# homenc/HElib

Hardware: AMD Instinct MI355X
Metric: ctxt_x_ctxt_mults_per_sec_incl_relinearize (higher is better)
Workload: dtype u64; 1 GPU; BGV m=32768 p=65537 bits=950 (L=16x60b, K=6x56b, 6 small primes, D=3): Ctxt::multiplyBy on FRESH ciphertexts = multLowLvl (bringToSet x2 + tensorProduct) + reLinearize (dropSmallAndSpecialPrimes + key switch), benchmarks/bgv_basic.cpp:144-165; added noise MEASURED as in the reference (device canonical-embedding norms, read back lazily); the loop is driven by the C++17 host (libhelib_amd_host.so); ; batch_per_gpu=128, pairs_all_ranks=128

## Files before the change

helib_amd/csrc/bgv_slots.hip:

```cpp
#include <hip/hip_runtime.h>

#include <cstdarg>
#include <cstdio>
#include <cstring>
#include <mutex>
#include <vector>

#include "../../include/helib_amd.h"
#include "bgv_slots.h"
#include "ckks_bridge.h"
#include "hostmath.h"
#include "prof.h"

struct hx_bgv_slots {
  hx_ctx* ctx = nullptr;
  hx_ctx* side = nullptr;
  uint64_t m = 0, p = 0, rho = 0, k = 0;
  uint32_t N = 0;
  int device = 0;
  std::vector<uint64_t> gens, ords;
  uint32_t* d_row2slot = nullptr;
  uint32_t* d_slot2row = nullptr;
  void* buf[3] = {nullptr, nullptr, nullptr};
  size_t cap[3] = {0, 0, 0};
// ... 76 lines not shown
    if (!best)
      break;
    gens.push_back(best);
    ords.push_back(largest);
    conj_classes(cl, best, m);
  }
}

int ensure_buf(hx_bgv_slots* t, hipStream_t st, int slot, size_t bytes)
{
  if (t->cap[slot] >= bytes)
    return HX_OK;
  CK(hipStreamSynchronize(st));
  hipFree(t->buf[slot]);
  t->buf[slot] = nullptr;
  t->cap[slot] = 0;
  CK(hipMalloc(&t->buf[slot], bytes));
  t->cap[slot] = bytes;
  return HX_OK;
}

struct Enter {
  hxi::CtxView v{};
  std::unique_lock<std::recursive_mutex> lk;
  int open(const hx_bgv_slots* t, const char* what)
  {
    RC(hxi::ctx_enter(t->ctx, &v));
    lk = std::unique_lock<std::recursive_mutex>(*v.mu);
    if (v.capturing)
      return err(HX_ERR_INVALID, "%s waits for the device and cannot be captured in a graph", what);
    return hx_ctx_set_stream(t->side, (void*)v.stream);
  }
};
struct DrainOnExit {
  hipStream_t st;
  ~DrainOnExit() { (void)hipStreamSynchronize(st); }
};
struct Drop {
  hx_poly* t;
  ~Drop() { hx_poly_destroy(t); }
};

unsigned blocks_for(size_t items)
{
  const size_t b = (items + 255) / 256;
  return (unsigned)std::min<size_t>(std::max<size_t>(b, 1), hx::BGV_MAX_BLOCKS);
}
bool aligned16(const void* a) { return ((uintptr_t)a & 15) == 0; }

int side_poly(const hx_bgv_slots* t, int batch, hx_poly** out)
{
  const int zero = 0;
  return hx_poly_create_uninit(t->side, batch, &zero, 1, out);
}

int gather_out(hx_bgv_slots* t, hipStream_t st, hx_poly* sp, size_t words, int64_t* slots_out)
{
  RC(ensure_buf(t, st, 2, words * 8));
  HX_LAUNCH(hx::bgv_gather_kernel, dim3(blocks_for(words)), dim3(256), 0, st, hxi::poly_rows_read(sp), t->d_slot2row, t->N,
            words, (int64_t*)t->buf[2]);
  CK(hipGetLastError());
  CK(hipMemcpyAsync(slots_out, t->buf[2], words * 8, hipMemcpyDeviceToHost, st));
  CK(hipStreamSynchronize(st));
  return HX_OK;
}

int launch_redmul(const hx_bgv_slots* t, hipStream_t st, const int64_t* src, size_t words, uint64_t f, uint64_t* dst)
{
  const uint64_t p = t->p, mu = (uint64_t)(((hxh::u128)1 << 64) / p), fs = hxh::shoup(f, p);
  if (words % 2 == 0 && aligned16(src) && aligned16(dst))
    HX_LAUNCH(hx::bgv_redmul_kernel<2>, dim3(blocks_for(words / 2)), dim3(256), 0, st, src, words, p, mu, f, fs, dst);
  else
    HX_LAUNCH(hx::bgv_redmul_kernel<1>, dim3(blocks_for(words)), dim3(256), 0, st, src, words, p, mu, f, fs, dst);
  CK(hipGetLastError());
  return HX_OK;
}

}

extern "C" int hx_bgv_slots_destroy(hx_bgv_slots* t)
{
  if (!t)
    return HX_OK;
  (void)hipSetDevice(t->device);
  if (t->side)
    hx_ctx_destroy(t->side);
  hipFree(t->d_row2slot);
  hipFree(t->d_slot2row);
  for (void* b : t->buf)
    hipFree(b);
  delete t;
  return HX_OK;
}

extern "C" int hx_bgv_slots_create(hx_ctx* ctx, uint64_t p, hx_bgv_slots** out)
{
  if (!ctx || !out)
    return err(HX_ERR_INVALID, "null argument");
  *out = nullptr;
  hxi::CtxView v{};
  RC(hxi::ctx_enter(ctx, &v));
  std::unique_lock<std::recursive_mutex> lk(*v.mu);
  if (v.capturing)
    return err(HX_ERR_INVALID, "hx_bgv_slots_create while a graph is being captured");
  const uint64_t m = v.m;
  if (p < 2 || p >= (1ull << 60) || !hxh::is_prime(p))
    return err(HX_ERR_INVALID, "the plaintext modulus p = %llu is not a prime below 2^60", (unsigned long long)p);
  if (m % p == 0)
    return err(HX_ERR_INVALID, "p = %llu divides m = %llu", (unsigned long long)p, (unsigned long long)m);
  if (p % m != 1) {
    uint64_t d = 1;
    for (uint64_t x = p % m; x != 1; x = x * (p % m) % m)
      d++;
    return err(HX_ERR_UNSUPPORTED,
               "d = ord_m(p) = %llu for p = %llu, m = %llu: only d = 1 (p = 1 mod m, slots in Z_p) is built",
               (unsigned long long)d, (unsigned long long)p, (unsigned long long)m);
  }
  const bool pow2 = (m & (m - 1)) == 0;
  if (pow2 ? (m < 16 || m > (1u << 17)) : (m < 3))
    return err(HX_ERR_UNSUPPORTED, "BGV slots on the device need a power-of-two m in [16, 2^17] or another m >= 3 (m = %llu)",
               (unsigned long long)m);
  if (!pow2 && m % 2 == 0 && (p - 1) % (2 * m) != 0)
    return err(HX_ERR_UNSUPPORTED, "even m = %llu that is not a power of two needs 2m | p - 1 (p = %llu)",
               (unsigned long long)m, (unsigned long long)p);
  hx_bgv_slots* t = new hx_bgv_slots();
  struct Guard {
    hx_bgv_slots* t;
    ~Guard() { hx_bgv_slots_destroy(t); }
  } guard{t};
  t->ctx = ctx;
  t->m = m;
  t->p = p;
  t->N = v.phim;
  t->device = v.device;
  RC(hx_ctx_create(&t->side, v.device, m));
  RC(hx_ctx_set_stream(t->side, (void*)v.stream));
  int pidx = -1;
  uint64_t root = 0;
  RC(hx_ctx_add_prime(t->side, p, 0, &pidx));
  RC(hx_ctx_prime(t->side, pidx, nullptr, &root));
  const uint64_t zeta = pow2 ? root : hxh::mulmod(root, root, p);
  std::vector<uint32_t> zidx(m, hx::BGV_NO_SLOT);
  uint32_t n = 0;
  uint64_t pw = 1;
  for (uint64_t j = 0; j < m; j++, pw = hxh::mulmod(pw, zeta, p))
    if (hxh::gcd(j, m) == 1) {
      zidx[j] = n++;
      if (pw > t->rho) {
        t->rho = pw;
        t->k = j;
      }
    }
  if (n != t->N || hxh::powmod(zeta, m, p) != 1)
    return err(HX_ERR_DEVICE, "internal: the transform's root for p = %llu is not an m-th root of unity", (unsigned long long)p);
  find_generators(m, t->gens, t->ords);
  uint64_t nslots = 1;
  for (uint64_t o : t->ords)
    nslots *= o;
  if (nslots != t->N)
    return err(HX_ERR_DEVICE, "internal: the hypercube of Z_%llu^* has %llu points, not phi(m)", (unsigned long long)m,
               (unsigned long long)nslots);
  std::vector<uint32_t> slot2row(t->N), row2slot(t->N, hx::BGV_NO_SLOT);
  const size_t ng = t->gens.size();
  std::vector<uint64_t> e(ng, 0), part(ng + 1, 1);
  for (uint32_t i = 0; i < t->N; i++) {
    const uint64_t ti = part[ng];
    const uint64_t pos = hxh::mulmod(t->k, hxh::invmod(ti, m), m);
// ... 169 lines not shown
```

helib_amd/csrc/conv_kernels.hip:

```cpp
#include "dev_common.h"
#include "conv_dev.h"
#include "ntt_kernel_util.h"
#include "prof.h"

namespace hx {

__device__ __forceinline__ uint64_t uniform_u64(uint64_t v)
{
  const uint32_t lo = (uint32_t)__builtin_amdgcn_readfirstlane((int)(uint32_t)v);
  const uint32_t hi = (uint32_t)__builtin_amdgcn_readfirstlane((int)(uint32_t)(v >> 32));
  return ((uint64_t)hi << 32) | lo;
}
__device__ __forceinline__ TW uniform_tw(const TW& t)
{
  TW r;
  r.w = uniform_u64(t.w);
  r.wp = uniform_u64(t.wp);
  return r;
}

template <uint32_t SRC, uint32_t DST>
struct ConvIO {
  static constexpr int LOAD_BOUND = 1;
  static constexpr bool LAZY_STORE = true;
// ... 97 lines not shown
  using RN = RowNTT<LOGN, AR>;
  uint64_t v[32];
  uint32_t nl[32];
  const unsigned w = wave_index();
  RN::template fwd<0>(fresh_tid(w), v, nl, lds, io, twf, q);
  __syncthreads();
  RN::template fwd<1>(fresh_tid(w), v, nl, lds, io, twf, q);
  __syncthreads();
  RN::template fwd<2>(fresh_tid(w), v, nl, lds, io, twf, q);
  __syncthreads();
  RN::template fwd<3>(fresh_tid(w), v, nl, lds, io, twf, q);
  __syncthreads();
  RN::template fwd<4>(fresh_tid(w), v, nl, lds, io, twf, q);
  __syncthreads();
  RN::template fwd<5>(fresh_tid(w), v, nl, lds, io, twf, q);
  __syncthreads();
  RN::template fwd<6>(fresh_tid(w), v, nl, lds, io, twf, q);
  __syncthreads();
  RN::template fwd<7>(fresh_tid(w), v, nl, lds, io, twf, q);
  __syncthreads();
  RN::template inv<0>(fresh_tid(w), v, nl, lds, io, twi, q);
  __syncthreads();
  RN::template inv<1>(fresh_tid(w), v, nl, lds, io, twi, q);
  __syncthreads();
  RN::template inv<2>(fresh_tid(w), v, nl, lds, io, twi, q);
  __syncthreads();
  RN::template inv<3>(fresh_tid(w), v, nl, lds, io, twi, q);
  __syncthreads();
  RN::template inv<4>(fresh_tid(w), v, nl, lds, io, twi, q);
  __syncthreads();
  RN::template inv<5>(fresh_tid(w), v, nl, lds, io, twi, q);
  __syncthreads();
  RN::template inv<6>(fresh_tid(w), v, nl, lds, io, twi, q);
  __syncthreads();
  RN::template inv<7>(fresh_tid(w), v, nl, lds, io, twi, q);
}

template <int LOGN, uint32_t SRC, uint32_t DST>
__global__ void __launch_bounds__(Geo<LOGN>::T, HX_NTT_MINWAVES(LOGN))
ntt_conv_kernel(ConvRowArgs A, ConvRows R, const PrimeDev* __restrict__ cprimes, const TW* __restrict__ tw_arena)
{
  extern __shared__ __attribute__((aligned(16))) uint32_t lds[];
  const unsigned wid = xcd_remap(blockIdx.x, gridDim.x);
  const unsigned b = wid % A.batch, u = wid / A.batch, ri = u / A.split, g = u % A.split;
  const PrimeDev* pd = cprimes + uniform_u16(R.pd, u);
  const BluePrimeDev* P = R.bp[ri];
  constexpr unsigned Q = Geo<LOGN>::N;
  ConvIO<SRC, DST> io;
  const size_t seg = (size_t)ri * A.batch + b;
  const size_t polyseg = ((size_t)uniform_u16(R.row, ri) * A.batch + b) * A.phim;
  io.src = SRC == CONV_SRC_REV ? A.in + seg * A.in_stride : A.in + polyseg;
  io.dst = DST == CONV_DST_SUB ? A.out + ((size_t)u * A.batch + b) * Q : A.out + polyseg;
  io.aux = DST == CONV_DST_FINAL ? A.aux + seg * A.aux_stride : nullptr;
  io.hat = R.hat[ri] + (size_t)g * Q;
  io.P = P;
  io.S = &R.cp[ri]->S;
  io.zidx = A.zidx;
  io.g = g;
  io.split = A.split;
  io.Q = Q;
  io.phim = A.phim;
  io.m = A.m;
  io.d = A.d;
  io.base = A.base;
  io.alias = A.alias;
  io.r2 = pd->r2;
  const QC q = make_qc(pd->q, pd->mu64);
  const TW* twf = tw_arena + pd->tw_fwd_off;
  const TW* twi = tw_arena + pd->tw_inv_off;
#ifndef HX_NO_PROTH
  if (pd->proth) {
    conv_body<LOGN, ArProth>(lds, io, reinterpret_cast<const TWM*>(twf), reinterpret_cast<const TWM*>(twi), q);
    return;
  }
#endif
  conv_body<LOGN, ArShoup>(lds, io, twf, twi, q);
}

template <int LOGN, uint32_t SRC, uint32_t DST>
static hipError_t launch_conv(const ConvRowArgs& A, const ConvRows& R, int nunits, const PrimeDev* cprimes,
                              const TW* tw_arena, hipStream_t st)
{
  constexpr size_t lds_bytes = (size_t)Geo<LOGN>::LDS_WORDS * 4;
  bool attr_set = false;
  if (!attr_set) {
    hipError_t e = hxp::dyn_lds((const void*)ntt_conv_kernel<LOGN, SRC, DST>,
                                       hipFuncAttributeMaxDynamicSharedMemorySize, (int)lds_bytes);
    if (e != hipSuccess)
      return e;
    attr_set = true;
  }
  HX_LAUNCH((ntt_conv_kernel<LOGN, SRC, DST>), dim3((unsigned)nunits * A.batch), dim3(Geo<LOGN>::T), lds_bytes, st, A, R,
            cprimes, tw_arena);
  return hipGetLastError();
}
template <int LOGN>
static hipError_t launch_conv_n(const ConvRowArgs& A, const ConvRows& R, int nunits, const PrimeDev* cprimes,
                                const TW* tw_arena, hipStream_t st)
{
  if (A.src_mode == CONV_SRC_BLUE_PRE && A.dst_mode == CONV_DST_SUB)
    return launch_conv<LOGN, CONV_SRC_BLUE_PRE, CONV_DST_SUB>(A, R, nunits, cprimes, tw_arena, st);
  if (A.src_mode == CONV_SRC_SCATTER && A.dst_mode == CONV_DST_SUB)
    return launch_conv<LOGN, CONV_SRC_SCATTER, CONV_DST_SUB>(A, R, nunits, cprimes, tw_arena, st);
  if (A.src_mode == CONV_SRC_REV && A.dst_mode == CONV_DST_SUB)
    return launch_conv<LOGN, CONV_SRC_REV, CONV_DST_SUB>(A, R, nunits, cprimes, tw_arena, st);
  if (A.src_mode == CONV_SRC_REV && A.dst_mode == CONV_DST_FINAL)
    return launch_conv<LOGN, CONV_SRC_REV, CONV_DST_FINAL>(A, R, nunits, cprimes, tw_arena, st);
  return hipErrorInvalidValue;
}
hipError_t launch_conv_rows(int logn, const ConvRowArgs& A, const ConvRows& R, int nunits, const PrimeDev* cprimes,
                            const TW* tw_arena, hipStream_t st)
{
  switch (logn) {
    case 13: return launch_conv_n<13>(A, R, nunits, cprimes, tw_arena, st);
    case 14: return launch_conv_n<14>(A, R, nunits, cprimes, tw_arena, st);
    case 15: return launch_conv_n<15>(A, R, nunits, cprimes, tw_arena, st);
  }
  return hipErrorInvalidValue;
}

}
```

helib_amd/csrc/engine.hip:

```cpp
#include <hip/hip_runtime.h>

#include <cstdarg>
#include <cstdio>
#include <cstdlib>
#include <cstring>
#include <algorithm>
#include <chrono>
#include <map>
#include <mutex>
#include <string>
#include <unordered_set>
#include <vector>

#include "../../include/helib_amd.h"
#include "arena.h"
#include "prof.h"
#include "switches.h"
#include "dev_common.h"
#include "hostmath.h"
#include "bluestein.h"
#include "pfa_dev.h"
#include "rns_kernels.h"
#include "mfma_ext.h"
#include "rns_mfma_dev.h"
// ... 156 lines not shown
  uint64_t* scratch[11] = {nullptr, nullptr, nullptr, nullptr, nullptr, nullptr, nullptr, nullptr, nullptr, nullptr, nullptr};
  uint32_t* d_redo = nullptr;
  size_t redo_cap = 0;
  size_t scratch_words[11] = {0, 0, 0, 0, 0, 0, 0, 0, 0, 0, 0};
  uint64_t aux_q[3] = {0, 0, 0};
  int bk = 0, n1 = 0, n2 = 0, n3 = 0;
  uint32_t dq = 0, mpad = 0;
  PrimeDev* d_cprimes = nullptr;
  int ncprimes = 0, cprimes_cap = 0;
  std::vector<struct BluePrime*> blue;
  uint16_t* d_pfa_idx = nullptr;
  std::vector<ConvPlan> bigplan;
  std::vector<int64_t> psi_low, phi_coef;
  std::map<std::vector<uint64_t>, ExtPlan*> plans;
  hxa::SlabArena arena;
  std::unordered_set<struct hx_poly*> polys;
  int refs = 1;
  std::recursive_mutex mu;
  double* d_frac = nullptr;
  size_t frac_cap = 0, frac_pos = 0;
  bool want_frac = false;
  int xs_first = 0, xs_rows = 0;
  double xs_inv_qd = 0;
  bool want_fdelta = false;
  double2* d_wtab = nullptr;
  double2 *d_bn_v = nullptr, *d_bn_w = nullptr, *d_bn_chat = nullptr, *d_bn_Z = nullptr;
  size_t bn_rows_cap = 0;
  unsigned long long* d_norm2 = nullptr;
  size_t norm_cap = 0;
  double2* d_norm_park = nullptr;
  size_t norm_park_cap = 0;
  struct NormPending {
    hipEvent_t ev;
    unsigned long long* pinned;
    size_t cap;
    int rows;
    double* out;
    bool slab;
  };
  std::vector<void*> norm_slabs;
  bool defer_norms = false;
  std::vector<NormPending> norm_pending, norm_free;
  hipStream_t norm_stream = nullptr;
  hipEvent_t norm_in_ev = nullptr, norm_out_ev = nullptr;
  bool norm_reads_xs = false, norm_reads_frac = false;
  hipEvent_t timer[2] = {nullptr, nullptr};
  bool capturing = false;
  int graphs_alive = 0;
  hipStream_t own_stream = nullptr;
  std::vector<void*> graph_retired;
  void* ckks = nullptr;
  void (*ckks_free)(void*) = nullptr;
  void* linalg = nullptr;
  void (*linalg_free)(void*) = nullptr;
};

struct hx_poly {
  hx_ctx* ctx;
  int batch;
  int cap_rows;
  std::vector<int> prime_idx;
  uint64_t* d;
  bool owns;
  struct Share {
    int refs;
  };
  Share* share = nullptr;
  bool exposed = false;
  size_t row_words() const { return (size_t)batch * ctx->phim; }
  int nrows() const { return (int)prime_idx.size(); }
  bool shared() const { return share && share->refs > 1; }
};

struct hx_ksk {
  hx_ctx* ctx;
  int ndig;
  std::vector<int> row_idx;
  uint64_t* d_b;
  uint64_t* d_a;
};

static int use(hx_ctx* c)
{
  HIPCHK(hipSetDevice(c->device));
  return HX_OK;
}
#define CTX_ENTER(ctx)                                             \
  std::lock_guard<std::recursive_mutex> _ctx_lock((ctx)->mu);      \
  CHK(use(ctx))

#define NO_CAPTURE(ctx, what)                                                                      \
  do {                                                                                             \
    if ((ctx)->capturing)                                                                          \
      return fail(HX_ERR_INVALID, what " waits for the device and cannot be captured in a graph"); \
  } while (0)

static constexpr size_t POOL_LIMIT = (size_t)64 << 30;
template <bool TRACE>
static int arena_sys_alloc_t(size_t bytes, void** out)
{
  const bool trace = TRACE;
  const auto t0 = std::chrono::steady_clock::now();
  hipError_t e = hipMalloc(out, bytes);
  if (trace)
    fprintf(stderr, "[helib_amd arena] hipMalloc(%zu MiB) took %.2f ms\n", bytes >> 20,
            std::chrono::duration<double, std::milli>(std::chrono::steady_clock::now() - t0).count());
  if (e != hipSuccess)
    (void)hipGetLastError();
  return (int)e;
}
static void arena_sys_free(void* p) { hipFree(p); }
static hipError_t pool_alloc(hx_ctx* c, size_t bytes, void** out)
{
  if (!c->arena.sys_alloc) {
    c->arena.sys_alloc = c->sw.arena_trace ? arena_sys_alloc_t<true> : arena_sys_alloc_t<false>;
    c->arena.sys_free = arena_sys_free;
  }
  int rc = c->arena.alloc(bytes, c->capturing, out);
  if (rc != 0 && !c->capturing) {
    (void)hipGetLastError();
    hipStreamSynchronize(c->stream);
    if (c->arena.trim(0) > 0)
      rc = c->arena.alloc(bytes, false, out);
  }
  return (hipError_t)rc;
}
static void retire_or_free(hx_ctx* c, void* p, bool device_wide_sync = false)
{
  if (!p)
    return;
  if (c->norm_stream)
    hipStreamSynchronize(c->norm_stream);
  if (c->capturing || c->graphs_alive > 0) {
    c->graph_retired.push_back(p);
    return;
  }
  if (device_wide_sync)
    hipDeviceSynchronize();
  else
    hipStreamSynchronize(c->stream);
  hipFree(p);
}
static void pool_free(hx_ctx* c, void* p, size_t bytes)
{
  (void)bytes;
  if ((c->capturing || c->graphs_alive > 0) && c->arena.is_pinned(p)) {
    c->arena.defer(p);
    return;
  }
  c->arena.release(p);
  if (c->arena.cached() > POOL_LIMIT && !c->capturing) {
    hipStreamSynchronize(c->stream);
    c->arena.trim(POOL_LIMIT / 2);
  }
}

static int norm_join(hx_ctx* c, bool xs, bool frac)
{
  if ((xs && c->norm_reads_xs) || (frac && c->norm_reads_frac)) {
    HIPCHK(hipStreamWaitEvent(c->stream, c->norm_out_ev, 0));
    c->norm_reads_xs = c->norm_reads_frac = false;
  }
  return HX_OK;
}

static int ensure_scratch(hx_ctx* c, int slot, size_t words)
{
// ... 15 lines not shown
{
  if (words == 0 || dst == src)
    return HX_OK;
  if (((uintptr_t)dst | (uintptr_t)src) & 15) {
    HIPCHK(hipMemcpyAsync(dst, src, words * 8, hipMemcpyDeviceToDevice, c->stream));
    return HX_OK;
  }
  const size_t blocks = std::min<size_t>((words / 2 + 255) / 256, (size_t)256 * 16);
  HX_LAUNCH(hx::copy_words_kernel, dim3((unsigned)std::max<size_t>(blocks, 1)), dim3(256), 0, c->stream,
                     dst, src, words);
  HIPCHK(hipGetLastError());
  return HX_OK;
}

static void storage_release(hx_poly* p)
{
  if (!p->owns || !p->d)
    return;
  const size_t bytes = (size_t)p->cap_rows * p->row_words() * 8;
  if (p->share) {
    if (--p->share->refs == 0) {
      pool_free(p->ctx, p->d, bytes);
      delete p->share;
    }
    p->share = nullptr;
  } else {
    pool_free(p->ctx, p->d, bytes);
  }
  p->d = nullptr;
}
static int poly_own(hx_poly* p)
{
  if (!p->share)
    return HX_OK;
  if (p->share->refs == 1) {
    delete p->share;
    p->share = nullptr;
    return HX_OK;
  }
  hx_ctx* c = p->ctx;
  uint64_t* nd = nullptr;
  const size_t bytes = (size_t)p->cap_rows * p->row_words() * 8;
  hipError_t e = pool_alloc(c, bytes, (void**)&nd);
  if (e != hipSuccess)
    return fail(HX_ERR_NOMEM, "hipMalloc(%zu) failed: %s", bytes, hipGetErrorString(e));
  CHK(dcopy(c, nd, p->d, (size_t)p->nrows() * p->row_words()));
  p->share->refs--;
  p->share = nullptr;
  p->d = nd;
  return HX_OK;
}
#define OWN(p) CHK(poly_own(p))
static int poly_fresh(hx_poly* p, const uint64_t** old_rows)
{
  *old_rows = p->d;
  if (!p->share)
    return HX_OK;
  if (p->share->refs == 1) {
    delete p->share;
    p->share = nullptr;
    return HX_OK;
  }
  uint64_t* nd = nullptr;
  const size_t bytes = (size_t)p->cap_rows * p->row_words() * 8;
  hipError_t e = pool_alloc(p->ctx, bytes, (void**)&nd);
  if (e != hipSuccess)
    return fail(HX_ERR_NOMEM, "hipMalloc(%zu) failed: %s", bytes, hipGetErrorString(e));
  p->share->refs--;
  p->share = nullptr;
  p->d = nd;
  return HX_OK;
}

static void ctx_free(hx_ctx* c);
extern "C" int hx_ctx_create(hx_ctx** out, int device, uint64_t m)
{
  if (!out || m < 2 || m > (1ull << 24))
    return fail(HX_ERR_INVALID, "Bad Z_m^* modulus m (must be in [2, 2^24])");
  int ndev = 0;
  if (hipGetDeviceCount(&ndev) != hipSuccess || ndev <= 0)
    return fail(HX_ERR_DEVICE, "no HIP device available (this library has no CPU path)");
  if (device < 0 || device >= ndev)
    return fail(HX_ERR_INVALID, "device %d out of range [0,%d)", device, ndev);
  HIPCHK(hipSetDevice(device));
  hx_ctx* c = new hx_ctx();
  c->sw = hxs::read();
  struct Guard {
    hx_ctx* c;
    ~Guard()
    {
      if (c)
        ctx_free(c);
    }
  } guard{c};
  c->device = device;
  c->m = m;
  std::vector<int32_t> zidx((size_t)m, -1);
  for (uint64_t i = 1; i < m; i++)
    if (hxh::gcd(i, m) == 1) {
      zidx[i] = (int32_t)c->zms.size();
      c->zms.push_back((uint32_t)i);
    }
  c->phim = (uint32_t)c->zms.size();
  c->pow2 = (m & (m - 1)) == 0;
  if (c->pow2) {
    int l = 0;
    while ((1u << l) < c->phim)
      l++;
    c->logn = l;
  }
  HIPCHK(hipMalloc((void**)&c->d_zms, (size_t)c->phim * 4));
  HIPCHK(hipMalloc((void**)&c->d_zms_index, (size_t)m * 4));
  HIPCHK(hipMalloc((void**)&c->d_perm, (size_t)c->phim * 4));
  HIPCHK(hipMemcpy(c->d_zms, c->zms.data(), (size_t)c->phim * 4, hipMemcpyHostToDevice));
  HIPCHK(hipMemcpy(c->d_zms_index, zidx.data(), (size_t)m * 4, hipMemcpyHostToDevice));
  c->primes_cap = 1024;
  HIPCHK(hipMalloc((void**)&c->d_primes, sizeof(PrimeDev) * c->primes_cap));
  guard.c = nullptr;
  *out = c;
  return HX_OK;
}

static void ctx_release(hx_ctx* c)
{
  bool last;
  {
    std::lock_guard<std::recursive_mutex> lk(c->mu);
    last = --c->refs == 0;
  }
  if (last)
    ctx_free(c);
}
extern "C" int hx_ctx_destroy(hx_ctx* c)
{
  if (!c)
    return HX_OK;
  ctx_release(c);
  return HX_OK;
}
static void ctx_free(hx_ctx* c)
{
  hipSetDevice(c->device);
  hipDeviceSynchronize();
  if (c->ckks_free)
    c->ckks_free(c->ckks);
  if (c->linalg_free)
    c->linalg_free(c->linalg);
  if (c->d_tw)
    hipFree(c->d_tw);
  for (auto& kv : c->plans) {
    hipFree(kv.second->blob);
    hipFree(kv.second->blob_mfma);
    delete kv.second;
  }
  for (int i = 0; i < 11; i++)
    if (c->scratch[i])
      hipFree(c->scratch[i]);
  c->arena.destroy();
  if (c->norm_stream) {
    hipStreamDestroy(c->norm_stream);
    hipEventDestroy(c->norm_in_ev);
    hipEventDestroy(c->norm_out_ev);
  }
  if (c->own_stream)
    hipStreamDestroy(c->own_stream);
  for (void* q : c->graph_retired)
    hipFree(q);
  hipFree(c->d_redo);
  hipFree(c->d_frac);
  hipFree(c->d_wtab);
  hipFree(c->d_bn_v);
  hipFree(c->d_bn_w);
  hipFree(c->d_bn_chat);
  hipFree(c->d_bn_Z);
  hipFree(c->d_norm2);
  hipFree(c->d_norm_park);
  for (auto* v : {&c->norm_pending, &c->norm_free})
    for (auto& np : *v) {
      hipEventDestroy(np.ev);
      if (!np.slab)
        hipHostFree(np.pinned);
    }
  for (void* q : c->norm_slabs)
    hipHostFree(q);
  for (BluePrime* b : c->blue) {
    if (!b)
      continue;
    hipFree(b->dev);
    hipFree(b->d_powers);
    hipFree(b->d_ipowers);
    hipFree(b->d_pfa);
    for (int i = 0; i < 5; i++) {
      hipFree(b->d_hat[i]);
      hipFree(b->d_hatw[i]);
    }
    for (int i = 0; i < 4; i++)
      hipFree(b->conv[i].dev);
    for (int j = 0; j < 3; j++) {
      for (int i = 0; i < 4; i++)
        hipFree(b->d_ahat[j][i]);
      for (int i = 0; i < 3; i++)
        hipFree(b->aconv[j][i].dev);
    }
    delete b;
  }
  if (c->d_cprimes)
    hipFree(c->d_cprimes);
  for (hipEvent_t e : c->timer)
    if (e)
      hipEventDestroy(e);
  hipFree(c->d_pfa_idx);
  hipFree(c->d_zms);
  hipFree(c->d_zms_index);
  hipFree(c->d_perm);
  hipFree(c->d_primes);
  delete c;
}

extern "C" int hx_ctx_phim(const hx_ctx* c, uint64_t* phim)
{
  if (!c || !phim)
    return fail(HX_ERR_INVALID, "null argument");
  *phim = c->phim;
  return HX_OK;
}
extern "C" int hx_ctx_set_stream(hx_ctx* c, void* s)
{
  if (!c)
    return fail(HX_ERR_INVALID, "null context");
  std::lock_guard<std::recursive_mutex> lk(c->mu);
  if (c->capturing)
    return fail(HX_ERR_INVALID, "hx_ctx_set_stream while a graph is being captured");
  if (c->stream != (hipStream_t)s) {
    hipSetDevice(c->device);
    hipStreamSynchronize(c->stream);
    if (c->norm_stream)
      hipStreamSynchronize(c->norm_stream);
  }
  c->stream = (hipStream_t)s;
  return HX_OK;
}
extern "C" int hx_ctx_sync(hx_ctx* c)
{
  if (!c)
    return fail(HX_ERR_INVALID, "null context");
  CTX_ENTER(c);
  NO_CAPTURE(c, "hx_ctx_sync");
  HIPCHK(hipStreamSynchronize(c->stream));
  if (c->norm_stream)
    HIPCHK(hipStreamSynchronize(c->norm_stream));
  return HX_OK;
}
extern "C" int hx_ctx_reserve(hx_ctx* c, uint64_t bytes)
{
  if (!c)
    return fail(HX_ERR_INVALID, "null context");
  CTX_ENTER(c);
  if (!c->arena.sys_alloc) {
    c->arena.sys_alloc = c->sw.arena_trace ? arena_sys_alloc_t<true> : arena_sys_alloc_t<false>;
    c->arena.sys_free = arena_sys_free;
  }
  const int rc = c->arena.reserve((size_t)bytes);
  if (rc != 0)
    return fail(HX_ERR_NOMEM, "hipMalloc(%llu) failed: %s", (unsigned long long)bytes, hipGetErrorString((hipError_t)rc));
  return HX_OK;
}
extern "C" int hx_ctx_arena_stats(hx_ctx* c, uint64_t out[4])
{
  if (!c || !out)
    return fail(HX_ERR_INVALID, "null argument");
  std::lock_guard<std::recursive_mutex> lk(c->mu);
  out[0] = c->arena.reserved;
  out[1] = c->arena.in_use;
  out[2] = c->arena.sys_calls;
  out[3] = c->arena.deferred.size();
  return HX_OK;
}
extern "C" int hx_ctx_num_primes(const hx_ctx* c, int* n)
{
  if (!c || !n)
    return fail(HX_ERR_INVALID, "null argument");
  *n = (int)c->primes.size();
  return HX_OK;
}
extern "C" int hx_ctx_prime(const hx_ctx* c, int idx, uint64_t* q, uint64_t* root)
{
  if (!c)
    return fail(HX_ERR_INVALID, "prime index out of range");
  std::lock_guard<std::recursive_mutex> lk(const_cast<hx_ctx*>(c)->mu);
  if (idx < 0 || idx >= (int)c->primes.size())
    return fail(HX_ERR_INVALID, "prime index out of range");
  if (q)
    *q = c->primes[idx].q;
  if (root)
    *root = c->primes[idx].root;
  return HX_OK;
}

static int tw_reserve(hx_ctx* c, size_t extra)
{
  if (c->tw_used + extra <= c->tw_cap)
    return HX_OK;
  size_t ncap = c->tw_cap ? c->tw_cap * 2 : extra * 32;
  while (ncap < c->tw_used + extra)
    ncap *= 2;
  TW* nd = nullptr;
  HIPCHK(hipMalloc((void**)&nd, ncap * sizeof(TW)));
  if (c->d_tw) {
    HIPCHK(hipDeviceSynchronize());
    HIPCHK(hipMemcpy(nd, c->d_tw, c->tw_used * sizeof(TW), hipMemcpyDeviceToDevice));
    retire_or_free(c, c->d_tw, true);
  }
  c->d_tw = nd;
  c->tw_cap = ncap;
  return HX_OK;
}

// ... 861 lines not shown
  }
  if (idx_out)
    *idx_out = idx;
  return HX_OK;
}

static int check_rows(hx_ctx* c, const int* idx, int n, bool allow_dup = false)
{
  if (n < 0 || (n > 0 && !idx))
    return fail(HX_ERR_INVALID, "bad prime index list");
  for (int i = 0; i < n; i++) {
    if (idx[i] < 0 || idx[i] >= (int)c->primes.size())
      return fail(HX_ERR_INVALID, "prime index %d not in the context", idx[i]);
    if (!allow_dup)
      for (int j = 0; j < i; j++)
        if (idx[j] == idx[i])
          return fail(HX_ERR_INVALID, "duplicate prime index %d", idx[i]);
  }
  return HX_OK;
}

static int poly_new(hx_ctx* c, int batch, const int* idx, int nrows, int cap, void* wrap,
                    bool allow_dup, hx_poly** out, bool zero = true)
{
  if (!c || !out || batch < 1)
    return fail(HX_ERR_INVALID, "bad argument");
  CTX_ENTER(c);
  CHK(check_rows(c, idx, nrows, allow_dup));
  if (cap < nrows)
    cap = nrows;
  if (cap < 1)
    cap = 1;
  if (!wrap)
    cap += 2;
  hx_poly* p = new hx_poly();
  p->ctx = c;
  p->batch = batch;
  p->cap_rows = cap;
  p->prime_idx.assign(idx, idx + nrows);
  p->owns = wrap == nullptr;
  if (wrap) {
    p->d = (uint64_t*)wrap;
  } else {
    size_t bytes = (size_t)cap * batch * c->phim * 8;
    hipError_t e = pool_alloc(c, bytes, (void**)&p->d);
    if (e != hipSuccess) {
      delete p;
      return fail(HX_ERR_NOMEM, "hipMalloc(%zu) failed: %s", bytes, hipGetErrorString(e));
    }
    e = zero ? hipMemsetAsync(p->d, 0, (size_t)nrows * batch * c->phim * 8, c->stream) : hipSuccess;
    if (e != hipSuccess) {
      pool_free(c, p->d, bytes);
      delete p;
      return fail(HX_ERR_DEVICE, "hipMemsetAsync failed: %s", hipGetErrorString(e));
    }
  }
  c->refs++;
  c->polys.insert(p);
  *out = p;
  return HX_OK;
}

extern "C" int hx_poly_create(hx_ctx* c, int batch, const int* idx, int nrows, hx_poly** out)
{
  return poly_new(c, batch, idx, nrows, nrows, nullptr, false, out);
}
extern "C" int hx_poly_create_uninit(hx_ctx* c, int batch, const int* idx, int nrows, hx_poly** out)
{
  return poly_new(c, batch, idx, nrows, nrows, nullptr, false, out, false);
}
extern "C" int hx_poly_wrap(hx_ctx* c, int batch, const int* idx, int nrows, void* dptr,
                            hx_poly** out)
{
  if (!dptr)
    return fail(HX_ERR_INVALID, "null device pointer");
  return poly_new(c, batch, idx, nrows, nrows, dptr, false, out);
}
extern "C" int hx_poly_destroy(hx_poly* p)
{
  if (!p)
    return HX_OK;
  {
    std::lock_guard<std::recursive_mutex> lk(p->ctx->mu);
    hipSetDevice(p->ctx->device);
    storage_release(p);
    p->ctx->polys.erase(p);
  }
  ctx_release(p->ctx);
  delete p;
  return HX_OK;
}
extern "C" int hx_poly_shape(const hx_poly* p, int* batch, int* nrows, uint64_t* phim)
{
  if (!p)
    return fail(HX_ERR_INVALID, "null poly");
  if (batch)
    *batch = p->batch;
  if (nrows)
    *nrows = p->nrows();
  if (phim)
    *phim = p->ctx->phim;
  return HX_OK;
}
extern "C" int hx_poly_primes(const hx_poly* p, int* out)
{
  if (!p || !out)
    return fail(HX_ERR_INVALID, "null argument");
  for (int i = 0; i < p->nrows(); i++)
    out[i] = p->prime_idx[i];
  return HX_OK;
}
extern "C" void* hx_poly_device_ptr(hx_poly* p)
{
  if (!p)
    return nullptr;
  std::lock_guard<std::recursive_mutex> lk(p->ctx->mu);
  hipSetDevice(p->ctx->device);
  if (poly_own(p) != HX_OK)
    return nullptr;
  p->exposed = true;
  return p->d;
}

extern "C" int hx_poly_upload(hx_poly* p, const uint64_t* host)
{
  if (!p || !host)
    return fail(HX_ERR_INVALID, "null argument");
  CTX_ENTER(p->ctx);
  NO_CAPTURE(p->ctx, "hx_poly_upload");
  OWN(p);
  size_t bytes = (size_t)p->nrows() * p->row_words() * 8;
  HIPCHK(hipMemcpyAsync(p->d, host, bytes, hipMemcpyHostToDevice, p->ctx->stream));
  HIPCHK(hipStreamSynchronize(p->ctx->stream));
  return HX_OK;
}
extern "C" int hx_poly_download(const hx_poly* p, uint64_t* host)
{
  if (!p || !host)
    return fail(HX_ERR_INVALID, "null argument");
  CTX_ENTER(p->ctx);
  NO_CAPTURE(p->ctx, "hx_poly_download");
  size_t bytes = (size_t)p->nrows() * p->row_words() * 8;
  HIPCHK(hipMemcpyAsync(host, p->d, bytes, hipMemcpyDeviceToHost, p->ctx->stream));
  HIPCHK(hipStreamSynchronize(p->ctx->stream));
  return HX_OK;
}

static int poly_reserve(hx_poly* p, int cap, bool keep = true)
{
  if (cap <= p->cap_rows)
    return HX_OK;
  if (!p->owns)
    return fail(HX_ERR_NOMEM, "wrapped poly has no room for %d rows", cap);
  hx_ctx* c = p->ctx;
  uint64_t* nd = nullptr;
  cap += 2;
  size_t bytes = (size_t)cap * p->row_words() * 8;
  hipError_t e = pool_alloc(c, bytes, (void**)&nd);
  if (e != hipSuccess)
    return fail(HX_ERR_NOMEM, "hipMalloc(%zu) failed: %s", bytes, hipGetErrorString(e));
  if (keep && p->nrows() > 0)
    CHK(dcopy(c, nd, p->d, (size_t)p->nrows() * p->row_words()));
  storage_release(p);
  p->d = nd;
  p->cap_rows = cap;
  return HX_OK;
}

extern "C" int hx_poly_copy(hx_poly* dst, const hx_poly* src)
{
  if (!dst || !src || dst->ctx != src->ctx || dst->batch != src->batch)
    return fail(HX_ERR_INVALID, "Context mismatch");
  CTX_ENTER(dst->ctx);
  if (dst == src)
    return HX_OK;
  hx_ctx* cc = dst->ctx;
  const bool lazy_ok = !cc->capturing && cc->graphs_alive == 0 && !dst->exposed && !src->exposed;
  if (dst->owns && src->owns && lazy_ok) {
    hx_poly* s = const_cast<hx_poly*>(src);
    if (dst->d == s->d)
      return HX_OK;
    storage_release(dst);
    if (!s->share)
      s->share = new hx_poly::Share{1};
    s->share->refs++;
    dst->share = s->share;
    dst->d = s->d;
    dst->cap_rows = s->cap_rows;
    dst->prime_idx = s->prime_idx;
    return HX_OK;
  }
  OWN(dst);
  CHK(poly_reserve(dst, src->nrows(), false));
  dst->prime_idx = src->prime_idx;
  CHK(dcopy(dst->ctx, dst->d, src->d, (size_t)src->nrows() * src->row_words()));
  return HX_OK;
}
extern "C" int hx_poly_set_zero(hx_poly* p)
{
  if (!p)
// ... 300 lines not shown
    return;
  const bool parked = !c->arena.deferred.empty() || !c->graph_retired.empty();
  if (parked)
    hipStreamSynchronize(c->stream);
  c->arena.unpin_all();
  for (void* q : c->graph_retired)
    hipFree(q);
  c->graph_retired.clear();
}
extern "C" int hx_ctx_graph_begin(hx_ctx* c)
{
  if (!c)
    return fail(HX_ERR_INVALID, "null context");
  CTX_ENTER(c);
  if (c->capturing)
    return fail(HX_ERR_INVALID, "a graph is already being captured on this context");
  if (!c->norm_pending.empty())
    return fail(HX_ERR_INVALID, "deferred norms are pending: hx_norms_flush before capturing");
  if (!c->stream) {
    HIPCHK(hipDeviceSynchronize());
    if (!c->own_stream)
      HIPCHK(hipStreamCreateWithFlags(&c->own_stream, hipStreamNonBlocking));
    c->stream = c->own_stream;
  }
  for (hx_poly* p : c->polys)
    if (p->share)
      CHK(poly_own(p));
  c->arena.pin_all();
  HIPCHK(hipStreamBeginCapture(c->stream, hipStreamCaptureModeRelaxed));
  c->capturing = true;
  return HX_OK;
}
extern "C" int hx_ctx_graph_end(hx_ctx* c, hx_graph** out)
{
  if (!c || !out)
    return fail(HX_ERR_INVALID, "null argument");
  CTX_ENTER(c);
  if (!c->capturing)
    return fail(HX_ERR_INVALID, "hx_ctx_graph_end without hx_ctx_graph_begin");
  c->capturing = false;
  hipGraph_t g = nullptr;
  hipError_t e = hipStreamEndCapture(c->stream, &g);
  if (e != hipSuccess || !g) {
    (void)hipGetLastError();
    graph_release_if_idle(c);
    return fail(HX_ERR_DEVICE, "graph capture failed (a captured call needed the device to finish?): %s",
                hipGetErrorString(e));
  }
  hipGraphExec_t x = nullptr;
  e = hipGraphInstantiate(&x, g, nullptr, nullptr, 0);
  if (e != hipSuccess) {
    (void)hipGetLastError();
    hipGraphDestroy(g);
    graph_release_if_idle(c);
    return fail(HX_ERR_DEVICE, "hipGraphInstantiate failed: %s", hipGetErrorString(e));
  }
  hx_graph* h = new hx_graph();
  h->ctx = c;
  h->graph = g;
  h->exec = x;
  c->graphs_alive++;
  c->refs++;
  *out = h;
  return HX_OK;
}
extern "C" int hx_graph_launch(hx_graph* g)
{
  if (!g)
    return fail(HX_ERR_INVALID, "null graph");
  hx_ctx* c = g->ctx;
  CTX_ENTER(c);
  if (c->capturing)
    return fail(HX_ERR_INVALID, "hx_graph_launch while another graph is being captured");
  HIPCHK(hipGraphLaunch(g->exec, c->stream));
  return HX_OK;
}
extern "C" int hx_graph_destroy(hx_graph* g)
{
  if (!g)
    return HX_OK;
  hx_ctx* c = g->ctx;
  {
    std::lock_guard<std::recursive_mutex> lk(c->mu);
    hipSetDevice(c->device);
    hipStreamSynchronize(c->stream);
    hipGraphExecDestroy(g->exec);
    hipGraphDestroy(g->graph);
    --c->graphs_alive;
    graph_release_if_idle(c);
  }
  ctx_release(c);
  delete g;
  return HX_OK;
}

static dim3 ew_grid(size_t row_words, int rows)
{
  size_t nvec = row_words / 2;
  size_t blocks = (nvec + 255) / 256;
  size_t cap = 8192 / (size_t)(rows > 0 ? rows : 1) + 1;
  if (blocks > cap)
    blocks = cap;
  if (blocks < 1)
    blocks = 1;
  return dim3((unsigned)blocks, (unsigned)rows);
}

template <int OP>
static int ew_binary(hx_poly* a, const hx_poly* b)
{
  if (!a || !b)
    return fail(HX_ERR_INVALID, "null poly");
  if (a->ctx != b->ctx)
    return fail(HX_ERR_INVALID, "DoubleCRT::Op: incompatible objects");
  if (b->batch != a->batch && b->batch != 1)
    return fail(HX_ERR_INVALID, "batch mismatch");
  CTX_ENTER(a->ctx);
  int rows = a->nrows();
  if (rows == 0)
    return HX_OK;
  if (rows > MAX_ROWS)
    return fail(HX_ERR_UNSUPPORTED, "too many rows");
  RowMap2 map;
  for (int r = 0; r < rows; r++) {
    int br = find_row(b->prime_idx, a->prime_idx[r]);
    if (br < 0)
      return fail(HX_ERR_PRIMESET, "DoubleCRT::Op: incompatible index sets (prime %d)",
                  a->prime_idx[r]);
    map.p[r] = (uint16_t)a->prime_idx[r];
    map.brow[r] = (uint16_t)br;
  }
  size_t rw = a->row_words();
  OWN(a);
  HX_LAUNCH((hx::ew_binary_kernel<OP>), ew_grid(rw, rows), dim3(256), 0, a->ctx->stream,
                     a->d, b->d, map, rw, b->row_words(), (int)(b->batch != a->batch),
                     (size_t)a->ctx->phim, a->ctx->d_primes);
  HIPCHK(hipGetLastError());
  return HX_OK;
}
extern "C" int hx_add(hx_poly* a, const hx_poly* b) { return ew_binary<hx::EW_ADD>(a, b); }
extern "C" int hx_sub(hx_poly* a, const hx_poly* b) { return ew_binary<hx::EW_SUB>(a, b); }
extern "C" int hx_mul(hx_poly* a, const hx_poly* b) { return ew_binary<hx::EW_MUL>(a, b); }

template <int OP>
static int ew_scalar_rows(hx_poly* a, const uint64_t* c_per_row, uint64_t exponent = 0)
{
  if (!a)
    return fail(HX_ERR_INVALID, "null poly");
  CTX_ENTER(a->ctx);
  int rows = a->nrows();
  if (rows == 0)
    return HX_OK;
  if (rows > MAX_ROWS)
    return fail(HX_ERR_UNSUPPORTED, "too many rows");
  RowMap map;
  RowScalars sc;
  for (int r = 0; r < rows; r++) {
    uint64_t q = a->ctx->primes[a->prime_idx[r]].q;
    map.p[r] = (uint16_t)a->prime_idx[r];
    uint64_t cv = c_per_row ? c_per_row[r] % q : 0;
    sc.c[r] = cv;
    sc.cp[r] = OP == hx::EWS_EXP ? exponent : hxh::shoup(cv, q);
  }
  size_t rw = a->row_words();
  OWN(a);
  HX_LAUNCH((hx::ew_scalar_kernel<OP>), ew_grid(rw, rows), dim3(256), 0, a->ctx->stream,
                     a->d, map, sc, rw, a->ctx->d_primes);
// ... 383 lines not shown
      uint8_t* dm = nullptr;
      HIPCHK(hipMalloc((void**)&dm, tab.size()));
      HIPCHK(hipMemcpy(dm, tab.data(), tab.size(), hipMemcpyHostToDevice));
      pl->blob_mfma = dm;
      pl->dev.mfma_a = dm;
      pl->dev.mfma_steps = (uint32_t)hx::mfx::steps_for(n);
    }
  }
  pl->dev.tgt_chunk7 = hx::as_ro(reinterpret_cast<const uint32_t*>(d + o_tchunk));
  {
    bool unit = scaled && ptxt > 1;
    for (int t = 0; t < nt && unit; t++)
      unit = ptxt <= tq(t);
    pl->dev.corr_unit = unit ? 1u : 0u;
  }
  c->plans[key] = pl;
  *out = pl;
  return HX_OK;
}

static int redo_prepare(hx_ctx* c, size_t row_words, uint32_t** out)
{
  const size_t need = row_words + 1;
  if (c->redo_cap < need) {
    uint32_t* nd = nullptr;
    HIPCHK(hipMalloc((void**)&nd, need * sizeof(uint32_t)));
    retire_or_free(c, c->d_redo);
    c->d_redo = nd;
    c->redo_cap = need;
  }
  HIPCHK(hipMemsetAsync(c->d_redo, 0, sizeof(uint32_t), c->stream));
  *out = c->d_redo;
  return HX_OK;
}
static int hps_min_n(const hx_ctx* c)
{
  return c->sw.hps_min_n;
}
static const dim3 REDO_GRID(64);

static int launch_extend(hx_ctx* c, const ExtPlan* pl, const ExtArgs& args_in, size_t row_words)
{
  dim3 grid((unsigned)((row_words + 255) / 256)), block(256);
  int n = pl->dev.n;
  ExtArgs args = args_in;
  args.redo = nullptr;
  if (pl->dev.fast16_ok) {
    const bool mfma = pl->dev.hps_ok && pl->dev.mfma_steps != 0 && args.upd == nullptr && row_words < ((size_t)1 << 32);
    const bool hps = mfma || (pl->dev.hps_ok && n >= hps_min_n(c) && args.upd == nullptr && row_words < ((size_t)1 << 32));
    if (hps)
      CHK(redo_prepare(c, row_words, &args.redo));
    if (mfma)
      HIPCHK(hx::launch_rns_extend_mfma(pl->dev, args, row_words, c->stream));
#define HX_EXT_FAST(NN)                                                                                            \
  case NN:                                                                                                         \
    if (hps) {                                                                                                     \
      if (!mfma)                                                                                                   \
        HX_LAUNCH((hx::rns_extend_fast_kernel<NN, true>), grid, block, 0, c->stream, pl->dev, args, row_words);    \
      HX_LAUNCH((hx::rns_extend_fast_kernel<NN, false>), REDO_GRID, block, 0, c->stream, pl->dev, args, row_words); \
    } else {                                                                                                       \
      HX_LAUNCH((hx::rns_extend_fast_kernel<NN, false>), grid, block, 0, c->stream, pl->dev, args, row_words);     \
    }                                                                                                              \
    break;
    switch (n) {
      HX_EXT_FAST(1) HX_EXT_FAST(2) HX_EXT_FAST(3) HX_EXT_FAST(4) HX_EXT_FAST(5) HX_EXT_FAST(6) HX_EXT_FAST(7) HX_EXT_FAST(8)
      HX_EXT_FAST(9) HX_EXT_FAST(10) HX_EXT_FAST(11) HX_EXT_FAST(12) HX_EXT_FAST(13) HX_EXT_FAST(14) HX_EXT_FAST(15)
      HX_EXT_FAST(16)
    }
#undef HX_EXT_FAST
    HIPCHK(hipGetLastError());
    return HX_OK;
  }
  const size_t wide_lds = (size_t)pl->dev.nt * (size_t)hx::wide_stride(n) * 8;
  if (pl->dev.wide_ok && row_words < ((size_t)1 << 32) && wide_lds <= 160 * 1024) {
    CHK(redo_prepare(c, row_words, &args.redo));
    if (pl->dev.mfma_steps) {
      HIPCHK(hx::launch_rns_extend_mfma(pl->dev, args, row_words, c->stream));
      HX_LAUNCH((hx::rns_extend_kernel<40>), REDO_GRID, block, 0, c->stream, pl->dev, args, row_words);
      HIPCHK(hipGetLastError());
      return HX_OK;
    }
    const dim3 wgrid((unsigned)((row_words + hx::WIDE_THREADS - 1) / hx::WIDE_THREADS)), wblock(hx::WIDE_THREADS);
    const size_t lds = wide_lds;
    static std::mutex wide_mu;
    static std::unordered_set<int> wide_attr;
    {
      std::lock_guard<std::mutex> lk(wide_mu);
      if (!wide_attr.count(c->device)) {
        for (const void* f : {(const void*)hx::rns_extend_wide_kernel<20>, (const void*)hx::rns_extend_wide_kernel<24>,
                              (const void*)hx::rns_extend_wide_kernel<28>, (const void*)hx::rns_extend_wide_kernel<32>,
                              (const void*)hx::rns_extend_wide_kernel<36>, (const void*)hx::rns_extend_wide_kernel<40>})
          HIPCHK(hxp::dyn_lds(f, 160 * 1024));
        wide_attr.insert(c->device);
      }
    }
    if (n <= 20)
      HX_LAUNCH((hx::rns_extend_wide_kernel<20>), wgrid, wblock, lds, c->stream, pl->dev, args, row_words);
    else if (n <= 24)
      HX_LAUNCH((hx::rns_extend_wide_kernel<24>), wgrid, wblock, lds, c->stream, pl->dev, args, row_words);
    else if (n <= 28)
      HX_LAUNCH((hx::rns_extend_wide_kernel<28>), wgrid, wblock, lds, c->stream, pl->dev, args, row_words);
    else if (n <= 32)
      HX_LAUNCH((hx::rns_extend_wide_kernel<32>), wgrid, wblock, lds, c->stream, pl->dev, args, row_words);
    else if (n <= 36)
      HX_LAUNCH((hx::rns_extend_wide_kernel<36>), wgrid, wblock, lds, c->stream, pl->dev, args, row_words);
    else
      HX_LAUNCH((hx::rns_extend_wide_kernel<40>), wgrid, wblock, lds, c->stream, pl->dev, args, row_words);
    HX_LAUNCH((hx::rns_extend_kernel<40>), REDO_GRID, block, 0, c->stream, pl->dev, args, row_words);
    HIPCHK(hipGetLastError());
    return HX_OK;
  }
  if (n <= 8)
    HX_LAUNCH((hx::rns_extend_kernel<8>), grid, block, 0, c->stream, pl->dev, args,
                       row_words);
  else if (n <= 16)
    HX_LAUNCH((hx::rns_extend_kernel<16>), grid, block, 0, c->stream, pl->dev, args,
                       row_words);
  else if (n <= 40)
    HX_LAUNCH((hx::rns_extend_kernel<40>), grid, block, 0, c->stream, pl->dev, args,
                       row_words);
  else if (n <= 64)
    HX_LAUNCH((hx::rns_extend_kernel<64>), grid, block, 0, c->stream, pl->dev, args,
                       row_words);
  else
    HX_LAUNCH((hx::rns_extend_kernel<MAX_EXT_SRC>), grid, block, 0, c->stream, pl->dev, args,
                       row_words);
  HIPCHK(hipGetLastError());
  return HX_OK;
}

static void clear_args(ExtArgs& a)
{
  memset(&a, 0xff, sizeof a);
  a.src = nullptr;
  a.dst = nullptr;
  a.upd = nullptr;
  a.nu = 0;
  a.frac = nullptr;
  a.redo = nullptr;
  a.lazy_out = 0;
}

static int bn_logp(const hx_ctx* c) { return next_pow2_exp(2 * c->m - 1); }

static int frac_begin(hx_ctx* c, size_t doubles)
{
  if (!c->pow2 && bn_logp(c) > 18)
    return fail(HX_ERR_UNSUPPORTED,
                "device embedding norms need m a power of two or m <= 131072 (otherwise the host keeps "
                "the reference's noiseBoundForUniform bound)");
  if (c->frac_cap < doubles) {
    CHK(norm_join(c, false, true));
    retire_or_free(c, c->d_frac);
    c->d_frac = nullptr;
    c->frac_cap = 0;
    HIPCHK(hipMalloc((void**)&c->d_frac, doubles * sizeof(double)));
    c->frac_cap = doubles;
  }
  CHK(norm_join(c, false, true));
  c->frac_pos = 0;
  c->want_frac = true;
  c->xs_rows = 0;
  return HX_OK;
}
static double* frac_take(hx_ctx* c, size_t doubles)
{
  if (!c->want_frac || c->frac_pos + doubles > c->frac_cap)
    return nullptr;
  double* p = c->d_frac + c->frac_pos;
  c->frac_pos += doubles;
  return p;
}

static int flush_xs(hx_ctx* c)
{
  if (c->xs_rows <= 0)
    return HX_OK;
  const size_t n = (size_t)c->xs_rows * c->phim;
  HX_LAUNCH(hx::frac_from_xs_kernel, dim3((unsigned)std::min<size_t>((n + 255) / 256, 4096)),
                     dim3(256), 0, c->stream, c->scratch[0],
                     reinterpret_cast<const int64_t*>(c->scratch[1]), c->xs_inv_qd,
                     c->d_frac + (size_t)c->xs_first * c->phim, n);
  HIPCHK(hipGetLastError());
  c->xs_rows = 0;
  return HX_OK;
}

static int bnorm_setup(hx_ctx* c)
{
  if (c->d_bn_chat)
    return HX_OK;
  const int bk = bn_logp(c);
  if (bk > 18)
    return fail(HX_ERR_UNSUPPORTED, "device embedding norms: m too large (2m-1 > 2^18)");
  const uint64_t m = c->m;
  const size_t P = (size_t)1 << bk;
  const long double pi = 3.141592653589793238462643383279502884L;
  std::vector<double> v(2 * m), cv(2 * P, 0.0), w(P);
  for (uint64_t k = 0; k < m; k++) {
    const uint64_t k2 = (uint64_t)(((hxh::u128)k * k) % (2 * m));
    const long double ang = pi * (long double)k2 / (long double)m;
    const double cr = (double)cosl(ang), si = (double)sinl(ang);
    v[2 * k] = cr;
    v[2 * k + 1] = si;
    cv[2 * k] = cr;
    cv[2 * k + 1] = -si;
    if (k) {
      cv[2 * (P - k)] = cr;
      cv[2 * (P - k) + 1] = -si;
    }
  }
  for (size_t k = 0; k < P / 2; k++) {
    const long double ang = 2 * pi * (long double)k / (long double)P;
    w[2 * k] = (double)cosl(ang);
    w[2 * k + 1] = (double)sinl(ang);
  }
  double2* d_cv = nullptr;
  HIPCHK(hipMalloc((void**)&c->d_bn_v, sizeof(double) * 2 * m));
  HIPCHK(hipMalloc((void**)&c->d_bn_w, sizeof(double) * P));
  HIPCHK(hipMalloc((void**)&c->d_bn_chat, sizeof(double) * 2 * P));
  HIPCHK(hipMalloc((void**)&d_cv, sizeof(double) * 2 * P));
  HIPCHK(hipMemcpy(c->d_bn_v, v.data(), sizeof(double) * 2 * m, hipMemcpyHostToDevice));
  HIPCHK(hipMemcpy(c->d_bn_w, w.data(), sizeof(double) * P, hipMemcpyHostToDevice));
  HIPCHK(hipMemcpy(d_cv, cv.data(), sizeof(double) * 2 * P, hipMemcpyHostToDevice));
  bool attr = false;
  if (!attr) {
    HIPCHK(hxp::dyn_lds((const void*)hx::bnorm_fwd_kernel, 16 << hx::NORM_MAX_LOGH));
    HIPCHK(hxp::dyn_lds((const void*)hx::bnorm_inv_kernel, 16 << hx::NORM_MAX_LOGH));
    attr = true;
  }
  const int logp = bk, logh = std::min(logp, hx::NORM_MAX_LOGH);
  const unsigned H = 1u << logh, S = (unsigned)(P >> logh);
  const unsigned threads = std::min<unsigned>(hx::NORM_THREADS, std::max<unsigned>(64u, H / 4));
  HX_LAUNCH(hx::bnorm_fwd_kernel, dim3(S), dim3(threads), std::max<size_t>(16 * (size_t)H, 256), c->stream,
                     (const double*)nullptr, (const double2*)nullptr, (const double2*)d_cv, c->d_bn_w,
                     (const double2*)nullptr, c->d_bn_chat, logp, logh, c->phim, 1);
  HIPCHK(hipGetLastError());
  HIPCHK(hipStreamSynchronize(c->stream));
  HIPCHK(hipFree(d_cv));
  return HX_OK;
}

static int embed_norms_general(hx_ctx* c, const double* d_f, int rows, hipStream_t ns)
{
  CHK(bnorm_setup(c));
  const int logp = bn_logp(c), logh = std::min(logp, hx::NORM_MAX_LOGH);
  const size_t P = (size_t)1 << logp;
  const unsigned H = 1u << logh, S = (unsigned)(P >> logh);
  const size_t cap = std::max<size_t>(1, ((size_t)1 << 28) / (16 * P));
  if (c->bn_rows_cap < std::min<size_t>(cap, (size_t)rows)) {
    retire_or_free(c, c->d_bn_Z);
    c->d_bn_Z = nullptr;
    c->bn_rows_cap = std::min<size_t>(cap, (size_t)rows);
    HIPCHK(hipMalloc((void**)&c->d_bn_Z, c->bn_rows_cap * P * 16));
  }
  const unsigned threads = std::min<unsigned>(hx::NORM_THREADS, std::max<unsigned>(64u, H / 4));
  const size_t lds = std::max<size_t>(16 * (size_t)H, 256);
  for (size_t r0 = 0; r0 < (size_t)rows; r0 += c->bn_rows_cap) {
    const unsigned nr = (unsigned)std::min<size_t>(c->bn_rows_cap, (size_t)rows - r0);
    HX_LAUNCH(hx::bnorm_fwd_kernel, dim3(nr * S), dim3(threads), lds, ns,
                       d_f + r0 * c->phim, (const double2*)c->d_bn_v, (const double2*)nullptr, c->d_bn_w,
                       (const double2*)c->d_bn_chat, c->d_bn_Z, logp, logh, c->phim, 0);
    HIPCHK(hipGetLastError());
    HX_LAUNCH(hx::bnorm_inv_kernel, dim3(nr * S), dim3(threads), lds, ns, c->d_bn_Z, c->d_bn_w,
                       logp, logh);
    HIPCHK(hipGetLastError());
    const unsigned gx = std::min<unsigned>(64u, (c->phim + 255u) / 256u);
    HX_LAUNCH(hx::bnorm_max_kernel, dim3(gx, nr), dim3(256), 0, ns, (const double2*)c->d_bn_Z,
                       c->d_bn_w, c->d_zms, c->phim, logp, logh, c->d_norm2 + r0);
    HIPCHK(hipGetLastError());
  }
  return HX_OK;
}

static int embed_norms(hx_ctx* c, const double* d_f, int rows, double* out_host)
{
  const uint32_t N = c->phim;
  const int logn = c->logn;
  if (c->pow2 && !c->d_wtab) {
    std::vector<double> h(2 * (size_t)N);
    const long double two_pi = 6.283185307179586476925286766559005768394L;
    for (uint32_t k = 0; k < N; k++) {
      long double ang = two_pi * (long double)k / (long double)c->m;
      h[2 * (size_t)k] = (double)cosl(ang);
      h[2 * (size_t)k + 1] = (double)sinl(ang);
    }
    HIPCHK(hipMalloc((void**)&c->d_wtab, sizeof(double) * 2 * (size_t)N));
    HIPCHK(hipMemcpy(c->d_wtab, h.data(), sizeof(double) * 2 * (size_t)N, hipMemcpyHostToDevice));
  }
  if (c->norm_cap < (size_t)rows) {
    retire_or_free(c, c->d_norm2);
    c->d_norm2 = nullptr;
    c->norm_cap = 0;
    HIPCHK(hipMalloc((void**)&c->d_norm2, sizeof(unsigned long long) * (size_t)rows));
    c->norm_cap = (size_t)rows;
  }
  const bool quarter_form = c->pow2 && logn >= 2 && logn - 1 <= hx::NORM_MAX_LOGH;
  const bool use_xs = quarter_form && c->xs_rows == rows && d_f == c->d_frac;
  if (!use_xs)
    CHK(flush_xs(c));
  hipStream_t ns = c->stream;
  const bool side_stream = c->sw.norm_async;
  if (side_stream && !c->capturing) {
    if (!c->norm_stream) {
      HIPCHK(hipStreamCreateWithFlags(&c->norm_stream, hipStreamNonBlocking));
      HIPCHK(hipEventCreateWithFlags(&c->norm_in_ev, hipEventDisableTiming));
      HIPCHK(hipEventCreateWithFlags(&c->norm_out_ev, hipEventDisableTiming));
    }
    HIPCHK(hipEventRecord(c->norm_in_ev, c->stream));
    HIPCHK(hipStreamWaitEvent(c->norm_stream, c->norm_in_ev, 0));
    ns = c->norm_stream;
  }
  hx_ctx::NormPending np{};
  bool have = false;
  for (size_t i = 0; i < c->norm_free.size(); i++)
    if (c->norm_free[i].cap >= (size_t)rows) {
      np = c->norm_free[i];
      c->norm_free.erase(c->norm_free.begin() + (long)i);
      have = true;
      break;
    }
  if (!have && rows <= 1024) {
    constexpr size_t PER = 64, CAP = 1024;
    unsigned long long* slab = nullptr;
    HIPCHK(hipHostMalloc((void**)&slab, PER * CAP * sizeof(unsigned long long), hipHostMallocDefault));
    c->norm_slabs.push_back(slab);
    for (size_t i = 0; i < PER; i++) {
      hx_ctx::NormPending f{};
      f.pinned = slab + i * CAP;
      f.cap = CAP;
      f.slab = true;
      HIPCHK(hipEventCreateWithFlags(&f.ev, hipEventDisableTiming));
      c->norm_free.push_back(f);
    }
    np = c->norm_free.back();
    c->norm_free.pop_back();
    have = true;
  }
  if (!have) {
    np.cap = (size_t)rows;
    np.slab = false;
    HIPCHK(hipHostMalloc((void**)&np.pinned, np.cap * sizeof(unsigned long long), hipHostMallocDefault));
    HIPCHK(hipEventCreateWithFlags(&np.ev, hipEventDisableTiming));
  }
  struct SlotGuard {
    hx_ctx* c;
    hx_ctx::NormPending* np;
    bool armed = true;
    ~SlotGuard()
    {
      if (armed)
        c->norm_free.push_back(*np);
    }
  } slot_guard{c, &np};
  const bool by_copy = c->sw.norm_memcpy;
  const bool r16_path = c->pow2 && !c->sw.norm_old && logn == 14;
  const bool x2_path = c->pow2 && logn == 15 && !c->sw.norm_old && !c->sw.norm_plain;
  const bool direct = !by_copy && (r16_path || x2_path);
  unsigned long long* const out2 = direct ? np.pinned : c->d_norm2;
  if (!direct)
    HIPCHK(hipMemsetAsync(c->d_norm2, 0, sizeof(unsigned long long) * (size_t)rows, ns));
  bool attr = false;
  if (!c->pow2) {
    CHK(flush_xs(c));
    CHK(embed_norms_general(c, d_f, rows, ns));
  } else if (!attr) {
    HIPCHK(hxp::dyn_lds((const void*)hx::embed_norm_kernel, 16 << hx::NORM_MAX_LOGH));
#define HX_NORM_ATTR(...)                                                                               \
  HIPCHK(hxp::dyn_lds((const void*)hx::embed_norm_quarter_kernel<__VA_ARGS__>,                   \
                             hipFuncAttributeMaxDynamicSharedMemorySize, 16 << hx::NORM_MAX_LOGH))
    HX_NORM_ATTR(hx::NormSrcF64, 0);
    HX_NORM_ATTR(hx::NormSrcF64, 13);
    HX_NORM_ATTR(hx::NormSrcF64, 14);
    HX_NORM_ATTR(hx::NormSrcXS, 0);
    HX_NORM_ATTR(hx::NormSrcXS, 13);
    HX_NORM_ATTR(hx::NormSrcXS, 14);
#undef HX_NORM_ATTR
    HIPCHK(hxp::dyn_lds((const void*)hx::embed_norm_quarter_split_kernel, 16 << hx::NORM_MAX_LOGH));
    attr = true;
  }
  if (!c->pow2) {
  } else if (logn >= 2 && logn - 1 <= hx::NORM_MAX_LOGH) {
    const unsigned M = N >> 1;
    const unsigned threads = std::min<unsigned>(hx::NORM_THREADS, std::max<unsigned>(64u, M / 4));
    const size_t lds = std::max<size_t>(16 * (size_t)M, 256);
    const bool full = threads == (unsigned)hx::NORM_THREADS;
#define HX_NORM_LAUNCH(SRCT, srcv)                                                                              \
  do {                                                                                                          \
    if (full && logn == 14)                                                                                     \
      HX_LAUNCH((hx::embed_norm_quarter_kernel<SRCT, 14>), dim3((unsigned)rows), dim3(threads), lds,   \
                         ns, srcv, c->d_wtab, logn, c->d_norm2);                                         \
    else if (full && logn == 13)                                                                                \
      HX_LAUNCH((hx::embed_norm_quarter_kernel<SRCT, 13>), dim3((unsigned)rows), dim3(threads), lds,   \
                         ns, srcv, c->d_wtab, logn, c->d_norm2);                                         \
    else                                                                                                        \
      HX_LAUNCH((hx::embed_norm_quarter_kernel<SRCT, 0>), dim3((unsigned)rows), dim3(threads), lds,    \
                         ns, srcv, c->d_wtab, logn, c->d_norm2);                                         \
  } while (0)
    const bool r16 = !c->sw.norm_old;
    constexpr size_t r16_lds = (size_t)hx::R16_LDS_DOUBLES * sizeof(double);
    if (r16 && logn == 14) {
      bool attr16 = false;
      if (!attr16) {
        HIPCHK(hxp::dyn_lds((const void*)hx::embed_norm_r16_kernel<hx::NormSrcXS>, (int)r16_lds));
        HIPCHK(hxp::dyn_lds((const void*)hx::embed_norm_r16_kernel<hx::NormSrcF64>, (int)r16_lds));
        attr16 = true;
      }
    }
    if (c->xs_rows == rows && d_f == c->d_frac) {
      hx::NormSrcXS src{c->scratch[0], reinterpret_cast<const int64_t*>(c->scratch[1]), c->xs_inv_qd};
      if (r16 && logn == 14)
        HX_LAUNCH((hx::embed_norm_r16_kernel<hx::NormSrcXS>), dim3((unsigned)rows), dim3(hx::R16_THREADS), r16_lds, ns, src,
                  c->d_wtab, out2, direct);
      else
        HX_NORM_LAUNCH(hx::NormSrcXS, src);
    } else {
      CHK(flush_xs(c));
      hx::NormSrcF64 src{d_f};
      if (r16 && logn == 14)
        HX_LAUNCH((hx::embed_norm_r16_kernel<hx::NormSrcF64>), dim3((unsigned)rows), dim3(hx::R16_THREADS), r16_lds, ns, src,
                  c->d_wtab, out2, direct);
      else
        HX_NORM_LAUNCH(hx::NormSrcF64, src);
    }
#undef HX_NORM_LAUNCH
    c->xs_rows = 0;
  } else if (logn - 1 > hx::NORM_MAX_LOGH && !c->sw.norm_plain) {
    CHK(flush_xs(c));
    const int logh = hx::NORM_MAX_LOGH;
    const unsigned H = 1u << logh, S = (N >> 1) >> logh;
    const size_t park_words = (size_t)rows * (S / 2) * H;
    const bool x2 = logn == 15 && !c->sw.norm_old;
    if (!x2 && c->norm_park_cap < park_words) {
      retire_or_free(c, c->d_norm_park);
      c->d_norm_park = nullptr;
      c->norm_park_cap = 0;
      HIPCHK(hipMalloc((void**)&c->d_norm_park, park_words * sizeof(double2)));
      c->norm_park_cap = park_words;
    }
    if (x2) {
      constexpr size_t x2_lds = 2 * (size_t)hx::R16_LDS_DOUBLES * sizeof(double);
      bool attrx2 = false;
      if (!attrx2) {
        HIPCHK(hxp::dyn_lds((const void*)hx::embed_norm_r16x2_kernel, (int)x2_lds));
        attrx2 = true;
      }
      HX_LAUNCH(hx::embed_norm_r16x2_kernel, dim3((unsigned)rows), dim3(2 * hx::R16_THREADS), x2_lds, ns, d_f, c->d_wtab,
                out2, direct);
    } else
    HX_LAUNCH(hx::embed_norm_quarter_split_kernel, dim3((unsigned)rows * (S / 2)), dim3(hx::NORM_THREADS),
                       16 * (size_t)H, ns, d_f, c->d_wtab, logn, logh, c->d_norm_park, c->d_norm2);
  } else {
    CHK(flush_xs(c));
    const int logh = std::min(logn, hx::NORM_MAX_LOGH);
    const unsigned H = 1u << logh, S = N >> logh;
    const unsigned threads = std::min<unsigned>(hx::NORM_THREADS, std::max<unsigned>(64u, H / 4));
    const size_t lds = std::max<size_t>(16 * (size_t)H, 256);
    HX_LAUNCH(hx::embed_norm_kernel, dim3((unsigned)rows * S), dim3(threads), lds, ns, d_f,
                       c->d_wtab, logn, logh, c->d_norm2);
  }
  HIPCHK(hipGetLastError());
  np.rows = rows;
  np.out = out_host;
  if (direct) {
  } else if (by_copy) {
    HIPCHK(hipMemcpyAsync(np.pinned, c->d_norm2, sizeof(unsigned long long) * (size_t)rows,
                          hipMemcpyDeviceToHost, ns));
  } else {
    HX_LAUNCH(hx::copy_words_kernel, dim3((unsigned)((rows + 255) / 256)), dim3(256), 0, ns,
              reinterpret_cast<uint64_t*>(np.pinned), reinterpret_cast<const uint64_t*>(c->d_norm2), (size_t)rows);
    HIPCHK(hipGetLastError());
  }
  HIPCHK(hipEventRecord(np.ev, ns));
  c->norm_pending.push_back(np);
  slot_guard.armed = false;
  if (ns != c->stream) {
    HIPCHK(hipEventRecord(c->norm_out_ev, ns));
    (use_xs ? c->norm_reads_xs : c->norm_reads_frac) = true;
  }
  if (c->defer_norms)
    return HX_OK;
  return hx_norms_flush(c);
}

static hipError_t wait_event(const hx_ctx* c, hipEvent_t ev)
{
  const auto t0 = std::chrono::steady_clock::now();
  for (;;) {
    for (int i = 0; i < 64; i++) {
      const hipError_t e = hipEventQuery(ev);
      if (e != hipErrorNotReady)
        return e;
    }
    if (std::chrono::steady_clock::now() - t0 > std::chrono::microseconds(c->sw.wait_poll_us))
      break;
  }
  return hipEventSynchronize(ev);
}

extern "C" int hx_norms_flush(hx_ctx* c)
{
  if (!c)
    return fail(HX_ERR_INVALID, "null context");
  CTX_ENTER(c);
  NO_CAPTURE(c, "hx_norms_flush");
  for (auto& np : c->norm_pending) {
    HIPCHK(wait_event(c, np.ev));
    for (int r = 0; r < np.rows; r++) {
      double v;
      memcpy(&v, &np.pinned[r], 8);
      np.out[r] = sqrt(v);
    }
    c->norm_free.push_back(np);
  }
  c->norm_pending.clear();
  return HX_OK;
}

extern "C" int hx_ctx_defer_norms(hx_ctx* c, int on)
{
  if (!c)
    return fail(HX_ERR_INVALID, "null context");
  c->defer_norms = on != 0;
  if (!on)
    return hx_norms_flush(c);
  return HX_OK;
}

extern "C" int hx_embedding_norm(hx_ctx* c, const double* f_host, int rows, double* norms_out)
// ... 883 lines not shown
  }
  if (owner_out)
    *owner_out = owner;
  return HX_OK;
}

static int break_digits_fused(hx_ctx* c, const uint64_t* coef, const std::vector<int>& own,
                              const int* dig_idx, const int* dig_off, int ndig,
                              const std::vector<int>& all, uint64_t* dig, size_t rw,
                              std::vector<int>* owner_out, bool lazy_out = false)
{
  const int L = (int)own.size(), nall = (int)all.size();
  if (ndig > hx::KS_MAXD || L > 64 || dig_off[ndig] != L)
    return HX_ERR_UNSUPPORTED;
  for (int r = 0; r < L; r++)
    if (all[r] != own[r] || dig_idx[r] != own[r])
      return HX_ERR_UNSUPPORTED;
  int nmax = 0;
  hx::BreakArgs A;
  memset(&A, 0, sizeof A);
  A.src = coef;
  A.dst = dig;
  A.L = L;
  A.nall = nall;
  A.ndig = ndig;
  std::vector<int> owner(nall, -1);
  for (int d = 0; d < ndig; d++) {
    A.off[d] = dig_off[d];
    int n = dig_off[d + 1] - dig_off[d];
    if (n < 1 || n > 16)
      return HX_ERR_UNSUPPORTED;
    nmax = std::max(nmax, n);
    std::vector<int> src(dig_idx + dig_off[d], dig_idx + dig_off[d + 1]), tgt;
    for (int r = 0; r < nall; r++) {
      if (r >= dig_off[d] && r < dig_off[d + 1])
        owner[r] = d;
      else
        tgt.push_back(all[r]);
    }
    ExtPlan* pl;
    CHK(get_plan(c, src, tgt, 0, &pl));
    A.plan[d] = pl->dev;
  }
  A.off[ndig] = dig_off[ndig];
  if (c->want_frac) {
    A.frac = frac_take(c, (size_t)ndig * rw);
    if (!A.frac)
      return fail(HX_ERR_INVALID, "internal: fraction buffer too small");
  }
  dim3 grid((unsigned)((rw + hx::BRK_THREADS - 1) / hx::BRK_THREADS)), block(hx::BRK_THREADS);
  size_t lds = (size_t)L * hx::BRK_THREADS * 8;
  bool fast = true;
  for (int d = 0; d < ndig; d++)
    fast = fast && A.plan[d].fast_ok;
  A.redo = nullptr;
  for (int d = 0; d < ndig; d++)
    lazy_out = lazy_out && A.plan[d].lazy_tight_ok;
  if (fast) {
    const int lds_rows = std::max(1, L - hx::break_fast_n0(A));
    for (const void* f : {(const void*)hx::break_digits_fast_kernel<true, false>, (const void*)hx::break_digits_fast_kernel<false, false>,
                          (const void*)hx::break_digits_fast_kernel<true, true>, (const void*)hx::break_digits_fast_kernel<false, true>})
      HIPCHK(hxp::dyn_lds(f, 64 * hx::BRK_THREADS * 8));
    const size_t lds_fast = (size_t)(lds_rows + std::max(0, std::min(40, c->sw.brk_lds_pad_rows))) * hx::BRK_THREADS * 8;
    bool hps = rw < ((size_t)1 << 32);
    for (int d = 0; d < ndig; d++)
      hps = hps && A.plan[d].hps_ok && (int)A.plan[d].n >= c->sw.brk_hps_min_n;
#define HX_BRK_LAUNCH(H, Z, G) HX_LAUNCH((hx::break_digits_fast_kernel<H, Z>), G, block, lds_fast, c->stream, A, rw)
    if (hps) {
      CHK(redo_prepare(c, rw, &A.redo));
      if (lazy_out) {
        HX_BRK_LAUNCH(true, true, grid);
        HX_BRK_LAUNCH(false, true, REDO_GRID);
      } else {
        HX_BRK_LAUNCH(true, false, grid);
        HX_BRK_LAUNCH(false, false, REDO_GRID);
      }
    } else if (lazy_out) {
      HX_BRK_LAUNCH(false, true, grid);
    } else {
      HX_BRK_LAUNCH(false, false, grid);
    }
#undef HX_BRK_LAUNCH
  } else if (nmax <= 8) {
    bool attr8 = false;
    if (!attr8) {
      HIPCHK(hxp::dyn_lds((const void*)hx::break_digits_kernel<8>, 64 * hx::BRK_THREADS * 8));
      attr8 = true;
    }
    HX_LAUNCH((hx::break_digits_kernel<8>), grid, block, lds, c->stream, A, rw);
  } else {
    bool attr16 = false;
    if (!attr16) {
      HIPCHK(hxp::dyn_lds((const void*)hx::break_digits_kernel<16>, 64 * hx::BRK_THREADS * 8));
      attr16 = true;
    }
    HX_LAUNCH((hx::break_digits_kernel<16>), grid, block, lds, c->stream, A, rw);
  }
  HIPCHK(hipGetLastError());
  if (owner_out)
    *owner_out = owner;
  return HX_OK;
}

static int build_all(const hx_poly* a, const int* sp_idx, int nsp, std::vector<int>& all)
{
  all = a->prime_idx;
  for (int i = 0; i < nsp; i++) {
    if (find_row(all, sp_idx[i]) >= 0)
      return fail(HX_ERR_PRIMESET,
                  "Special primes and CtxtPart's index set have non-empty intersection");
    all.push_back(sp_idx[i]);
  }
  return HX_OK;
}

extern "C" int hx_break_into_digits(const hx_poly* a, const int* dig_idx, const int* dig_off,
                                    int ndig, const int* sp_idx, int nsp, hx_poly* out)
{
  if (!a || !out || !dig_idx || !dig_off || ndig < 1)
    return fail(HX_ERR_INVALID, "bad argument");
  hx_ctx* c = a->ctx;
  if (out->ctx != c || out->batch != a->batch)
    return fail(HX_ERR_INVALID, "Context mismatch");
  CTX_ENTER(c);
  CHK(check_rows(c, sp_idx, nsp));
  std::vector<int> all;
  CHK(build_all(a, sp_idx, nsp, all));
  int nall = (int)all.size(), L = a->nrows();
  if (nall > MAX_ROWS)
    return fail(HX_ERR_UNSUPPORTED, "too many rows");
  size_t rw = a->row_words();
  OWN(out);
  CHK(poly_reserve(out, ndig * nall, out == a));
  out->prime_idx.clear();
  for (int d = 0; d < ndig; d++)
    out->prime_idx.insert(out->prime_idx.end(), all.begin(), all.end());
  CHK(ensure_scratch(c, 0, (size_t)L * rw));
  CHK(dcopy(c, c->scratch[0], a->d, (size_t)L * rw));
  CHK(ntt_rows(c, c->scratch[0], a->prime_idx, L, 0, L, a->batch, true));
  CHK(break_digits_coef(c, c->scratch[0], a->prime_idx, dig_idx, dig_off, ndig, all, out->d, rw));
  CHK(ntt_rows(c, out->d, all, nall, 0, ndig * nall, a->batch, false));
  return HX_OK;
}

extern "C" int hx_break_into_digits_norms(const hx_poly* a, const int* dig_idx, const int* dig_off,
                                          int ndig, const int* sp_idx, int nsp, hx_poly* out,
                                          double* norms)
{
  if (!a || !norms || ndig < 1)
    return fail(HX_ERR_INVALID, "bad argument");
  hx_ctx* c = a->ctx;
  CTX_ENTER(c);
  NO_CAPTURE(c, "hx_break_into_digits_norms (a norm read-back)");
  const size_t rw = a->row_words();
  CHK(frac_begin(c, (size_t)ndig * rw));
  int rc = hx_break_into_digits(a, dig_idx, dig_off, ndig, sp_idx, nsp, out);
  return finish_norms(c, rc, (size_t)ndig * rw, ndig * a->batch, norms, nullptr);
}

extern "C" int hx_ksk_create(hx_ctx* c, int ndig, const int* row_idx, int nrows, const uint64_t* b,
                             const uint64_t* a, hx_ksk** out)
{
  if (!c || !out || !b || !a || ndig < 1)
    return fail(HX_ERR_INVALID, "bad argument");
  CTX_ENTER(c);
  CHK(check_rows(c, row_idx, nrows));
  hx_ksk* k = new hx_ksk();
  struct Guard {
    hx_ksk* k;
    ~Guard()
    {
      if (k) {
        hipFree(k->d_b);
        hipFree(k->d_a);
        delete k;
      }
    }
  } guard{k};
  k->ctx = c;
  k->ndig = ndig;
  k->row_idx.assign(row_idx, row_idx + nrows);
  size_t bytes = (size_t)ndig * nrows * c->phim * 8;
  HIPCHK(hipMalloc((void**)&k->d_b, bytes));
  HIPCHK(hipMalloc((void**)&k->d_a, bytes));
  HIPCHK(hipMemcpy(k->d_b, b, bytes, hipMemcpyHostToDevice));
  HIPCHK(hipMemcpy(k->d_a, a, bytes, hipMemcpyHostToDevice));
  c->refs++;
  guard.k = nullptr;
  *out = k;
  return HX_OK;
}
extern "C" int hx_ksk_shape(const hx_ksk* k, int* ndig, int* nrows, int* row_idx_out)
{
  if (!k || !ndig || !nrows)
    return fail(HX_ERR_INVALID, "null argument");
  *ndig = k->ndig;
  *nrows = (int)k->row_idx.size();
  if (row_idx_out)
    for (size_t r = 0; r < k->row_idx.size(); r++)
      row_idx_out[r] = k->row_idx[r];
  return HX_OK;
}
extern "C" int hx_ksk_download(const hx_ksk* k, uint64_t* b, uint64_t* a)
{
  if (!k || !b || !a)
    return fail(HX_ERR_INVALID, "null argument");
  hx_ctx* c = k->ctx;
  CTX_ENTER(c);
  NO_CAPTURE(c, "hx_ksk_download (a synchronous copy)");
  const size_t bytes = (size_t)k->ndig * k->row_idx.size() * c->phim * 8;
  HIPCHK(hipStreamSynchronize(c->stream));
  HIPCHK(hipMemcpy(b, k->d_b, bytes, hipMemcpyDeviceToHost));
  HIPCHK(hipMemcpy(a, k->d_a, bytes, hipMemcpyDeviceToHost));
  return HX_OK;
}
extern "C" int hx_ksk_destroy(hx_ksk* k)
{
  if (!k)
    return HX_OK;
  hipSetDevice(k->ctx->device);
  hipStreamSynchronize(k->ctx->stream);
  hipFree(k->d_b);
  hipFree(k->d_a);
  ctx_release(k->ctx);
  delete k;
  return HX_OK;
}

static int tensor_launch(const hx_poly* c0, const hx_poly* c1, const hx_poly* d0,
                         const hx_poly* d1, uint64_t* o0, uint64_t* o1, uint64_t* o2,
                         const uint64_t* scale_per_row)
{
  hx_ctx* c = c0->ctx;
  int rows = c0->nrows();
  if (rows > MAX_ROWS)
    return fail(HX_ERR_UNSUPPORTED, "too many rows");
  const hx_poly* ps[3] = {c1, d0, d1};
  for (auto* p : ps)
    if (p->ctx != c || p->batch != c0->batch || p->prime_idx != c0->prime_idx)
      return fail(HX_ERR_PRIMESET,
                  "tensorProduct: parts must be defined relative to the same set of primes");
  RowMap map;
  RowScalars sc;
  memset(&sc, 0, sizeof sc);
  for (int r = 0; r < rows; r++) {
    map.p[r] = (uint16_t)c0->prime_idx[r];
    if (scale_per_row) {
      uint64_t q = c->primes[c0->prime_idx[r]].q;
      sc.c[r] = scale_per_row[r] % q;
      sc.cp[r] = hxh::shoup(sc.c[r], q);
    }
  }
  size_t rw = c0->row_words();
  HX_LAUNCH(hx::tensor_kernel, ew_grid(rw, rows), dim3(256), 0, c->stream, c0->d, c1->d,
                     d0->d, d1->d, o0, o1, o2, map, sc, scale_per_row ? 1 : 0, rw, c->d_primes);
  HIPCHK(hipGetLastError());
  return HX_OK;
}

extern "C" int hx_tensor(const hx_poly* c0, const hx_poly* c1, const hx_poly* d0,
                         const hx_poly* d1, hx_poly* o0, hx_poly* o1, hx_poly* o2)
{
  if (!c0 || !c1 || !d0 || !d1 || !o0 || !o1 || !o2)
    return fail(HX_ERR_INVALID, "null poly");
  CTX_ENTER(c0->ctx);
  hx_poly* os[3] = {o0, o1, o2};
  for (auto* o : os) {
    if (o->ctx != c0->ctx || o->batch != c0->batch)
      return fail(HX_ERR_INVALID, "Context mismatch");
    OWN(o);
    CHK(poly_reserve(o, c0->nrows(), false));
    o->prime_idx = c0->prime_idx;
  }
  return tensor_launch(c0, c1, d0, d1, o0->d, o1->d, o2->d, nullptr);
}

static int keyswitch_launch(hx_ctx* c, const uint64_t* dig, const hx_ksk* W,
                            const std::vector<int>& all, int batch, uint64_t* out0, uint64_t* out1,
                            int accumulate_rows, const uint64_t* own_src = nullptr,
                            const std::vector<int>* owner = nullptr,
                            const std::vector<std::vector<int>>* digit_primes = nullptr,
                            int ndig = -1, const uint64_t* t0s = nullptr, const uint64_t* t1s = nullptr,
                            const hx::TensorSrc* ts = nullptr)
{
  int nall = (int)all.size();
  if (ndig < 0)
    ndig = W->ndig;
  if (nall > MAX_ROWS)
    return fail(HX_ERR_UNSUPPORTED, "too many rows");
  RowMap2 map;
  for (int r = 0; r < nall; r++) {
    int wr = find_row(W->row_idx, all[r]);
    if (wr < 0)
      return fail(HX_ERR_PRIMESET, "key-switching matrix is not defined on the operand's primes");
    map.p[r] = (uint16_t)all[r];
    map.brow[r] = (uint16_t)wr;
  }
  size_t rw = (size_t)batch * c->phim;
  int lazy = W->ndig <= 8 ? 1 : 0;
  for (int r : all)
    if (hxh::bitlen(c->primes[r].q) > 60)
      lazy = 0;
  const hx::KsFix* d_fix = nullptr;
// ... 423 lines not shown
```

helib_amd/csrc/ntt_core.h:

```cpp
#pragma once
#include <stdint.h>
#include <utility>
#if defined(HX_CHECK_BOUNDS) && !defined(__HIP_DEVICE_COMPILE__)
#include <cstdio>
#include <cstdlib>
#include <type_traits>
#endif

#if defined(__HIPCC__)
#define HXD __host__ __device__ __forceinline__
#else
#define HXD inline
#endif

namespace hx {

struct TW {
  uint64_t w;
  uint64_t wp;
};

HXD uint64_t mulhi64(uint64_t a, uint64_t b)
{
#if defined(__HIP_DEVICE_COMPILE__)
// ... 641 lines not shown
                 "+v"(o[7]), "+v"(o[8]), "+v"(o[9]), "+v"(o[10]), "+v"(o[11]), "+v"(o[12]),
                 "+v"(o[13]), "+v"(o[14]), "+v"(o[15])
               :
               : "memory");
  asm volatile(""
               : "+v"(o[16]), "+v"(o[17]), "+v"(o[18]), "+v"(o[19]), "+v"(o[20]), "+v"(o[21]),
                 "+v"(o[22]), "+v"(o[23]), "+v"(o[24]), "+v"(o[25]), "+v"(o[26]), "+v"(o[27]),
                 "+v"(o[28]), "+v"(o[29]), "+v"(o[30]), "+v"(o[31])
               :
               : "memory");
}
#else
template <class Cst>
HXD void lds_read32(const uint32_t* lds, unsigned base, uint32_t (&o)[32])
{
  for (int e = 0; e < 32; e++)
    o[e] = lds[base + Cst::at(e)];
}
#endif
template <int LOGN>
struct CstAbB {
  static constexpr unsigned at(int e) { return 33u * ((unsigned)e << Geo<LOGN>::LC); }
};
template <int LOGN>
struct CstBcC {
  static constexpr unsigned at(int i)
  {
    return (unsigned)Geo<LOGN>::T * ((unsigned)i >> Geo<LOGN>::LC) + 1024u * ((unsigned)i & ((1u << Geo<LOGN>::LC) - 1u));
  }
};
template <int LOGN>
struct CstBcB {
  static constexpr unsigned at(int e) { return 32u * brev_bits((unsigned)e, 5); }
};
template <int LOGN>
struct CstAbA {
  static constexpr unsigned at(int e) { return brev_bits((unsigned)e, 5); }
};
HXD uint32_t half_of(uint64_t x, int half) { return half ? (uint32_t)(x >> 32) : (uint32_t)x; }
HXD void set_half(uint64_t& x, int half, uint32_t w)
{
  x = half ? ((x & 0xffffffffull) | ((uint64_t)w << 32)) : ((x & 0xffffffff00000000ull) | w);
}

template <int LOGN>
HXD unsigned coef_index(unsigned tid, int e) { return ((unsigned)e << (LOGN - 5)) + tid; }
template <int LOGN>
HXD unsigned eval_index(unsigned tid, int i)
{
  constexpr int LC = Geo<LOGN>::LC;
  constexpr int T = Geo<LOGN>::T;
  unsigned gi = (unsigned)i >> LC, ep = (unsigned)i & ((1u << LC) - 1u);
  return brev_bits(ep, LC) * 1024u + tid + (unsigned)T * gi;
}

template <int LOGN>
HXD unsigned coef_const(int e) { return (unsigned)e << (LOGN - 5); }
template <int LOGN>
HXD unsigned eval_const(int i)
{
  constexpr int LC = Geo<LOGN>::LC;
  constexpr int T = Geo<LOGN>::T;
  unsigned gi = (unsigned)i >> LC, ep = (unsigned)i & ((1u << LC) - 1u);
  return brev_bits(ep, LC) * 1024u + (unsigned)T * gi;
}

template <class IO, class = void>
struct io_skip_load : std::false_type {};
template <class IO>
struct io_skip_load<IO, std::void_t<decltype(IO::SKIP_LOAD)>> : std::integral_constant<bool, IO::SKIP_LOAD> {};

template <class IO, class AR, class = void>
struct io_load_bound : std::integral_constant<int, IO::LOAD_BOUND> {};
template <class IO, class AR>
struct io_load_bound<IO, AR, std::void_t<decltype(IO::template load_bound<AR>())>>
    : std::integral_constant<int, IO::template load_bound<AR>()> {};

template <class IO, class AR, class = void>
struct io_inv_load_bound : std::integral_constant<int, 1> {};
template <class IO, class AR>
struct io_inv_load_bound<IO, AR, std::void_t<decltype(IO::template inv_load_bound<AR>())>>
    : std::integral_constant<int, IO::template inv_load_bound<AR>()> {};

struct PtrIO {
  static constexpr int LOAD_BOUND = 1;
  static constexpr bool LAZY_STORE = false;
  static constexpr bool PIPELINED = false;
  struct StorePrefetch {};
  const uint64_t* in;
  uint64_t* out;
  HXD uint64_t load(unsigned tid, unsigned c) const { return in[tid + c]; }
  HXD void store(unsigned tid, unsigned c, uint64_t v) const { out[tid + c] = v; }
  HXD TW last_tw(TW def, int) const { return def; }
  HXD TWM last_tw(TWM def, int) const { return def; }
};

HXD uint64_t norm4(uint64_t x, uint64_t q, uint64_t q2)
{
  x = (x >= q2) ? x - q2 : x;
  return (x >= q) ? x - q : x;
}
HXD uint64_t norm2(uint64_t x, uint64_t q)
{
  return (x >= q) ? x - q : x;
}
template <int B, bool EST = false>
HXD uint64_t norm_from(uint64_t x, const QC& c)
{
  static_assert(B >= 1 && B <= 16, "bound");
  HX_BOUND(x, B, c.q);
  if constexpr (EST && B > 4) {
    const uint32_t xl = (uint32_t)x, xh = (uint32_t)(x >> 32);
    const uint64_t t = (uint64_t)xh * c.mu32 + mulhi32(xl, c.mu32);
    const uint32_t e = (uint32_t)(t >> 32);
    const uint32_t nl = (uint32_t)c.nq, nh = (uint32_t)(c.nq >> 32);
    uint64_t r = (uint64_t)e * nl + x;
    r += (uint64_t)(e * nh) << 32;
    HX_BOUND(r, 2, c.q);
    return csub(r, c.q);
  } else {
    if constexpr (B > 8)
      x = csub(x, c.q8);
    if constexpr (B > 4)
      x = csub(x, c.q4);
    if constexpr (B > 2)
      x = csub(x, c.q + c.q);
    if constexpr (B > 1)
      x = csub(x, c.q);
    return x;
  }
}

template <int LOGN, class AR = ArShoup>
struct RowNTT {
  using G = Geo<LOGN>;
  static constexpr int NPHASE = 8;


  template <int PH, class IO, class TWS>
  static HXD void fwd(unsigned tid, uint64_t (&v)[32], uint32_t (&nl)[32], uint32_t* lds,
                      const IO& io, const TWS& tw, const QC& c)
  {
    constexpr int LB = io_load_bound<IO, AR>::value;
    constexpr int L0 = LB * AR::U;
    constexpr int FA = pass_bound_out<AR, 5, false, 31, L0>();
    constexpr int FB = pass_bound_out<AR, 5, false, 31, FA>();
    constexpr int FCU = pass_bound_out<AR, G::LC, false, G::GC - 1, FB>();
    constexpr int FC = (FCU + AR::U - 1) / AR::U;
    static_assert(LB <= AR::FWD_LOAD_MAX && FA <= 16 * AR::U && FB <= 16 * AR::U && FCU <= 16 * AR::U, "lazy bounds");
    if constexpr (PH == 0) {
      if constexpr (IO::PIPELINED) {
        io.template load_all<LOGN, AR>(tid, v, c);
      } else {
#pragma unroll
        for (int e = 0; e < 32; e++) {
          v[e] = io.load(tid, coef_const<LOGN>(e));
          HX_IO_FENCE(e);
        }
      }
      run_pass<AR, 5, false, 1, 31, L0>(v, c, [&](int, int sp, int k, uint32_t) {
        return tw_uni(tw, (unsigned)((1 << sp) - 1 + k));
      });
#pragma unroll
      for (int e = 0; e < 32; e++)
        lds[ab_addr_A<LOGN>(tid, e)] = half_of(v[e], 0);
    } else if constexpr (PH == 1) {
// ... 37 lines not shown
        if (c.mu32)
          io.template store_all<LOGN, AR, FC, true>(tid, v, c, pre);
        else
          io.template store_all<LOGN, AR, FC, false>(tid, v, c, pre);
      } else if (c.mu32) {
#pragma unroll
        for (int i = 0; i < 32; i++) {
          io.store(tid, eval_const<LOGN>(i), norm_from<FC, true>(v[i], c));
          HX_IO_FENCE(i);
        }
      } else {
#pragma unroll
        for (int i = 0; i < 32; i++) {
          io.store(tid, eval_const<LOGN>(i), norm_from<FC, false>(v[i], c));
          HX_IO_FENCE(i);
        }
      }
    }
  }

  template <int PH, class IO, class TWS>
  static HXD void inv(unsigned tid, uint64_t (&v)[32], uint32_t (&nl)[32], uint32_t* lds,
                      const IO& io, const TWS& tw, const QC& c)
  {
    constexpr int I0 = io_inv_load_bound<IO, AR>::value;
    constexpr int IC_ = pass_bound_out<AR, G::LC, true, G::GC - 1, I0>();
    constexpr int IB = pass_bound_out<AR, 5, true, 31, IC_>();
    static_assert(I0 <= AR::inv_cap() && IC_ <= AR::inv_cap() && IB <= AR::inv_cap(), "lazy bounds");
    if constexpr (PH == 0) {
      if constexpr (!io_skip_load<IO>::value) {
#pragma unroll
        for (int i = 0; i < 32; i++)
          v[i] = io.load(tid, eval_const<LOGN>(i));
      }
      run_pass<AR, G::LC, true, G::NGC, G::GC - 1, I0>(v, c, [&](int gi, int sp, int k, uint32_t dep) {
        return tw_vec(tw, G::TWC, tid, ((1u << sp) - 1u + (unsigned)k) * 1024u + (unsigned)(G::T * gi), dep);
      });
#pragma unroll
      for (int i = 0; i < 32; i++)
        lds[bc_addr_C<LOGN>(tid, i)] = half_of(v[i], 0);
    } else if constexpr (PH == 1) {
      lds_read32<CstBcB<LOGN>>(lds, bc_addr_B<LOGN>(tid, 0), nl);
    } else if constexpr (PH == 2) {
#pragma unroll
      for (int i = 0; i < 32; i++)
        lds[bc_addr_C<LOGN>(tid, i)] = half_of(v[i], 1);
    } else if constexpr (PH == 3) {
      uint32_t nh[32];
      lds_read32<CstBcB<LOGN>>(lds, bc_addr_B<LOGN>(tid, 0), nh);
#pragma unroll
      for (int e = 0; e < 32; e++)
        v[e] = ((uint64_t)nh[e] << 32) | nl[e];
      run_pass<AR, 5, true, 1, 31, IC_>(v, c, [&](int, int sp, int k, uint32_t dep) {
        return tw_vec(tw, G::TWB, tid & 31u, ((1u << sp) - 1u + (unsigned)k) * 32u, dep);
      });
    } else if constexpr (PH == 4) {
#pragma unroll
      for (int e = 0; e < 32; e++)
        lds[ab_addr_B<LOGN>(tid, e)] = half_of(v[e], 0);
    } else if constexpr (PH == 5) {
      lds_read32<CstAbA<LOGN>>(lds, ab_addr_A<LOGN>(tid, 0), nl);
    } else if constexpr (PH == 6) {
#pragma unroll
      for (int e = 0; e < 32; e++)
        lds[ab_addr_B<LOGN>(tid, e)] = half_of(v[e], 1);
    } else if constexpr (PH == 7) {
      uint32_t nh[32];
      lds_read32<CstAbA<LOGN>>(lds, ab_addr_A<LOGN>(tid, 0), nh);
#pragma unroll
      for (int e = 0; e < 32; e++)
        v[e] = ((uint64_t)nh[e] << 32) | nl[e];
      run_pass<AR, 5, true, 1, 30, IB>(v, c, [&](int, int sp, int k, uint32_t) {
        return tw_uni(tw, (unsigned)((1 << sp) - 1 + k));
      });
      {
        const typename AR::Tw tS = io.last_tw(tw_uni(tw, 0), 0), tN = io.last_tw(tw_uni(tw, 31), 1);
        static_for<0, 16>([&](auto J) {
          constexpr int j = decltype(J)::value;
          AR::template gs_last<AR::inv_after(IB, 3, j)>(v[j], v[j + 16], tN, tS, c);
          if constexpr (HX_BF_FENCE > 0 && j % 2 == 1)
            HX_SCHED_FENCE();
        });
      }
#pragma unroll
      for (int e = 0; e < 32; e++) {
        io.store(tid, coef_const<LOGN>(e), norm_from<AR::INV_OUT>(v[e], c));
        HX_IO_FENCE(e);
      }
    }
  }
};

template <int LOGN, class MulMod>
inline void build_tw_tables_sub(uint64_t q, uint64_t psi, uint64_t psi_inv, uint64_t n_inv,
                                MulMod mulmod, int OUT, unsigned g, TW* fwd, TW* inv)
{
  using G = Geo<LOGN>;
  const int FULL = LOGN + OUT;
  const int NF = 1 << FULL;
  uint64_t* pw = new uint64_t[NF];
  uint64_t* ipw = new uint64_t[NF];
  pw[0] = ipw[0] = 1;
  for (int i = 1; i < NF; i++) {
    pw[i] = mulmod(pw[i - 1], psi, q);
    ipw[i] = mulmod(ipw[i - 1], psi_inv, q);
  }
  auto mk = [&](uint64_t w) {
    TW t;
    t.w = w;
    t.wp = (uint64_t)((((unsigned __int128)w) << 64) / q);
    return t;
  };
  auto src = [&](unsigned idx) {
    int sp = 31 - __builtin_clz(idx);
    unsigned j = idx - (1u << sp);
    unsigned full = (((1u << OUT) + g) << sp) + j;
    return brev_bits(full, FULL);
  };
  for (int i = 0; i < G::TW_TOTAL; i++) {
    fwd[i] = mk(0);
    inv[i] = mk(0);
  }
  for (int s = 0; s < 5; s++)
    for (int k = 0; k < (1 << s); k++) {
      unsigned e = src(twA_src<LOGN>(s, k));
      fwd[(1 << s) - 1 + k] = mk(pw[e]);
      inv[(1 << s) - 1 + k] = mk(ipw[e]);
    }
  inv[0] = mk(mulmod(ipw[src(1)], n_inv, q));
  inv[31] = mk(n_inv);
  for (int sp = 0; sp < 5; sp++)
    for (int k = 0; k < (1 << sp); k++)
      for (unsigned hip = 0; hip < 32; hip++) {
        unsigned e = src(twB_src<LOGN>(sp, k, hip));
        fwd[G::TWB + ((1 << sp) - 1 + k) * 32 + hip] = mk(pw[e]);
        inv[G::TWB + ((1 << sp) - 1 + k) * 32 + hip] = mk(ipw[e]);
      }
  for (int sp = 0; sp < G::LC; sp++)
    for (int k = 0; k < (1 << sp); k++)
      for (unsigned u = 0; u < 1024; u++) {
        unsigned e = src(twC_src<LOGN>(sp, k, u));
        fwd[G::TWC + ((1 << sp) - 1 + k) * 1024 + u] = mk(pw[e]);
        inv[G::TWC + ((1 << sp) - 1 + k) * 1024 + u] = mk(ipw[e]);
      }
  delete[] pw;
  delete[] ipw;
}

template <int LOGN, class MulMod>
inline void build_tw_tables(uint64_t q, uint64_t psi, uint64_t psi_inv, uint64_t n_inv,
                            MulMod mulmod, TW* fwd, TW* inv)
{
  build_tw_tables_sub<LOGN>(q, psi, psi_inv, n_inv, mulmod, 0, 0u, fwd, inv);
}
inline TWM tw_mont_form(uint64_t w, uint64_t q) { return (uint64_t)((((unsigned __int128)w) << 64) % q); }
inline void tw_tables_to_mont(const TW* t, int n, uint64_t q, TWM* out)
{
  for (int i = 0; i < n; i++)
    out[i] = tw_mont_form(t[i].w, q);
}

template <class MulMod>
inline void build_tw_small(int logn, uint64_t q, uint64_t psi, uint64_t psi_inv, uint64_t n_inv,
                           MulMod mulmod, TW* fwd, TW* inv)
{
  const int N = 1 << logn;
  uint64_t* pw = new uint64_t[N];
  uint64_t* ipw = new uint64_t[N];
  pw[0] = ipw[0] = 1;
  for (int i = 1; i < N; i++) {
// ... 22 lines not shown
```

helib_amd/csrc/ntt_kernels.hip:

```cpp
#include <cstdlib>
#include "dev_common.h"
#include "prof.h"

#include "ntt_kernel_util.h"

#ifdef HX_NTT_ONLY
#define HX_SFX2(n, s) n##_L##s
#define HX_SFX1(n, s) HX_SFX2(n, s)
#define HX_ENTRY(n) HX_SFX1(n, HX_NTT_ONLY)
#else
#define HX_ENTRY(n) n
#endif
#if !defined(HX_NTT_ONLY) || HX_NTT_ONLY == 13
#define HX_SZ_13(...) case 13: return __VA_ARGS__;
#else
#define HX_SZ_13(...)
#endif
#if !defined(HX_NTT_ONLY) || HX_NTT_ONLY == 14
#define HX_SZ_14(...) case 14: return __VA_ARGS__;
#else
#define HX_SZ_14(...)
#endif
#if !defined(HX_NTT_ONLY) || HX_NTT_ONLY == 15
#define HX_SZ_15(...) case 15: return __VA_ARGS__;
#else
#define HX_SZ_15(...)
#endif
#define HX_SZ(N, ...) HX_SZ_##N(__VA_ARGS__)

namespace hx {

typedef int v4i32 __attribute__((ext_vector_type(4)));
typedef int v2i32 __attribute__((ext_vector_type(2)));
__device__ v2i32 hx_buffer_load_v2(v4i32 rsrc, int voffset, int soffset,
                                   int aux) __asm("llvm.amdgcn.raw.buffer.load.v2i32");
__device__ void hx_buffer_store_v2(v2i32 data, v4i32 rsrc, int voffset, int soffset,
                                   int aux) __asm("llvm.amdgcn.raw.buffer.store.v2i32");

#ifdef HX_NO_NT
#define HX_NT 0
#define HX_NT_ASM ""
#else
#define HX_NT 2
#define HX_NT_ASM " nt"
#endif

__device__ v4i32 hx_buffer_load_v4(v4i32 rsrc, int voffset, int soffset,
                                   int aux) __asm("llvm.amdgcn.raw.buffer.load.v4i32");

__device__ __forceinline__ v4i32 make_rsrc(const uint64_t* row, unsigned bytes)
{
  uint64_t a = (uint64_t)row;
  v4i32 r;
  r.x = __builtin_amdgcn_readfirstlane((int)(uint32_t)a);
  r.y = __builtin_amdgcn_readfirstlane((int)(uint32_t)(a >> 32));
  r.z = (int)bytes;
  r.w = 0x00020000;
  return r;
}
struct BufTw {
  v4i32 r;
  const TW* p;
  __device__ explicit BufTw(const TW* tw) : r(make_rsrc(reinterpret_cast<const uint64_t*>(tw), 0xfffffff0u)), p(tw) {}
};
__device__ __forceinline__ TW tw_uni(const BufTw& t, unsigned i) { return t.p[i]; }
__device__ __forceinline__ TW tw_vec(const BufTw& t, unsigned base, unsigned lane, unsigned off, uint32_t dep)
{
  int vo = (int)(lane * 16u);
  asm volatile("" : "+v"(vo) : "v"(dep));
  const v4i32 x = hx_buffer_load_v4(t.r, vo, (int)((base + off) * 16u), 0);
  TW w;
  w.w = ((uint64_t)(uint32_t)x.y << 32) | (uint32_t)x.x;
  w.wp = ((uint64_t)(uint32_t)x.w << 32) | (uint32_t)x.z;
  return w;
}

template <int LB>
struct BufIOT {
  static constexpr int LOAD_BOUND = LB;
#ifndef HX_DIGITS_LB8
  template <class AR>
  static constexpr int load_bound() { return (LB == 8 && AR::PROTH) ? 2 : LB; }
#endif
  static constexpr bool LAZY_STORE = false;
  static constexpr bool PIPELINED = false;
  struct StorePrefetch {};
  v4i32 rin, rout;
  __device__ BufIOT(const uint64_t* in_row, uint64_t* out_row, unsigned bytes)
      : rin(make_rsrc(in_row, bytes)), rout(make_rsrc(out_row, bytes))
  {
  }
  __device__ __forceinline__ uint64_t load(unsigned tid, unsigned c) const
  {
    v2i32 r = hx_buffer_load_v2(rin, (int)(tid * 8u), (int)(c * 8u), HX_NT);
    return ((uint64_t)(uint32_t)r.y << 32) | (uint32_t)r.x;
  }
  __device__ __forceinline__ void store(unsigned tid, unsigned c, uint64_t v) const
  {
    v2i32 d;
    d.x = (int)(uint32_t)v;
    d.y = (int)(uint32_t)(v >> 32);
    hx_buffer_store_v2(d, rout, (int)(tid * 8u), (int)(c * 8u), HX_NT);
  }
  __device__ __forceinline__ TW last_tw(TW def, int) const { return def; }
  __device__ __forceinline__ TWM last_tw(TWM def, int) const { return def; }
};

struct InvPrepIO {
  static constexpr int LOAD_BOUND = 1;
  static constexpr bool LAZY_STORE = false;
  static constexpr bool PIPELINED = false;
  struct StorePrefetch {};
  v4i32 rin, rx;
  TW upS, upN;
  uint32_t has_up;
  __device__ InvPrepIO(const uint64_t* in_row, const ModDownPrep& p, size_t boff, unsigned bytes)
      : rin(make_rsrc(in_row, bytes)), rx(make_rsrc(p.xs + boff, bytes)), upS(p.upS), upN(p.upN),
        has_up(p.has_up)
  {
  }
  __device__ __forceinline__ uint64_t load(unsigned tid, unsigned c) const
  {
    v2i32 r = hx_buffer_load_v2(rin, (int)(tid * 8u), (int)(c * 8u), HX_NT);
    return ((uint64_t)(uint32_t)r.y << 32) | (uint32_t)r.x;
  }
  __device__ __forceinline__ void store(unsigned tid, unsigned c, uint64_t x) const
  {
    v2i32 d;
    d.x = (int)(uint32_t)x;
    d.y = (int)(uint32_t)(x >> 32);
    hx_buffer_store_v2(d, rx, (int)(tid * 8u), (int)(c * 8u), 0);
  }
  __device__ __forceinline__ TW last_tw(TW def, int which) const
  {
    return has_up ? (which ? upN : upS) : def;
  }
  __device__ __forceinline__ TWM last_tw(TWM def, int which) const
  {
    return has_up ? (which ? upN.wp : upS.wp) : def;
  }
};

__device__ __forceinline__ int64_t moddown_S_of(const ModDownPrep& P, uint64_t x)
{
  const bool neg = x > P.half;
  int64_t S = neg ? 1 : 0;
  if (P.ptxt > 1) {
    const uint64_t p = P.ptxt;
    uint64_t r = red64(x, p, P.ptxt_mu64);
    if (neg)
      r = sub_mod(r, P.qd_mod_p, p);
    if (r != 0) {
      const uint64_t dm = (p >> 32) == 0 ? red64(r * P.qdinv_mod_p, p, P.ptxt_mu64)
                                         : mul_mod(r, P.qdinv_mod_p, p, P.ptxt_mu, P.ptxt_k);
      const uint64_t p2 = p >> 1;
      const bool sub_p = dm > p2 || (((p & 1) == 0) && dm == p2 && neg);
      S += sub_p ? (int64_t)dm - (int64_t)p : (int64_t)dm;
    }
  }
  return S;
}
template <int UNUSED = 0>
__global__ void __launch_bounds__(256)
moddown_S_kernel(ModDownPrep P, size_t n2)
{
  const ulonglong2* xs = reinterpret_cast<const ulonglong2*>(P.xs);
  longlong2* S = reinterpret_cast<longlong2*>(P.S);
  for (size_t i = (size_t)blockIdx.x * blockDim.x + threadIdx.x; i < n2; i += (size_t)gridDim.x * blockDim.x) {
    const ulonglong2 x = xs[i];
    longlong2 s;
    s.x = moddown_S_of(P, x.x);
    s.y = moddown_S_of(P, x.y);
    S[i] = s;
  }
}

template <bool PLAIN>
struct ModDownIO {
  static constexpr int LOAD_BOUND = PLAIN ? 8 : 6;
  template <class AR>
#ifndef HX_DIGITS_LB8
  static constexpr int load_bound() { return AR::PROTH ? 4 : (PLAIN ? 8 : 6); }
#else
  static constexpr int load_bound() { return PLAIN ? 8 : (AR::PROTH ? 4 : 6); }
#endif
  static constexpr bool LAZY_STORE = true;
  static constexpr bool PIPELINED = !PLAIN;
  static constexpr int IOG = 4;
  struct StorePrefetch {
    uint64_t c[IOG];
  };
  v4i32 rx, rS, rc, ro;
  TW inv, cf;
  uint64_t q;
  __device__ ModDownIO(const uint64_t* x_row, const int64_t* S_row, const ModDownRow& R, const uint64_t* c_row,
                       uint64_t* o_row, unsigned bytes, uint64_t q_)
      : rx(make_rsrc(x_row, bytes)), rS(make_rsrc((const uint64_t*)S_row, bytes)),
        rc(make_rsrc(c_row, bytes)), ro(make_rsrc(o_row, bytes)), inv(R.inv), cf(R.cf), q(q_)
  {
  }
  __device__ __forceinline__ uint64_t load(unsigned tid, unsigned c) const
  {
    v2i32 a = hx_buffer_load_v2(rx, (int)(tid * 8u), (int)(c * 8u), HX_NT);
    return ((uint64_t)(uint32_t)a.y << 32) | (uint32_t)a.x;
  }
  static __device__ __forceinline__ uint64_t ld(const v4i32& r, unsigned tid, unsigned c)
  {
    v2i32 a = hx_buffer_load_v2(r, (int)(tid * 8u), (int)(c * 8u), 0);
    return ((uint64_t)(uint32_t)a.y << 32) | (uint32_t)a.x;
  }
  template <int LOGN, class AR>
  __device__ __forceinline__ void load_all(unsigned tid, uint64_t (&v)[32], const QC& qc) const
  {
    static_for<0, 32>([&](auto E) {
      constexpr int e = decltype(E)::value;
      v[e] = ld(rx, tid, coef_const<LOGN>(e));
    });
    uint64_t sb[2][IOG];
    static_for<0, IOG>([&](auto J) {
      constexpr int j = decltype(J)::value;
      sb[0][j] = ld(rS, tid, coef_const<LOGN>(j));
    });
    HX_SCHED_FENCE();
    static_for<0, 32 / IOG>([&](auto GI) {
      constexpr int g = decltype(GI)::value;
      if constexpr (g + 1 < 32 / IOG)
        static_for<0, IOG>([&](auto J) {
          constexpr int j = decltype(J)::value;
          sb[(g + 1) & 1][j] = ld(rS, tid, coef_const<LOGN>((g + 1) * IOG + j));
        });
      static_for<0, IOG>([&](auto J) {
        constexpr int j = decltype(J)::value, e = g * IOG + j;
        if constexpr (AR::PROTH)
          v[e] = mont_acc(v[e], inv.wp, qc, q - sb[g & 1][j]);
        else
          v[e] = shoup4_acc(v[e], inv, qc.nq, q - sb[g & 1][j]);
      });
      HX_SCHED_FENCE();
    });
  }
  static __device__ __forceinline__ uint64_t ld_pinned(const v4i32& r, unsigned tid, unsigned c)
  {
    uint64_t x;
    asm volatile("buffer_load_dwordx2 %0, %1, %2, %3 offen" HX_NT_ASM
                 : "=v"(x)
                 : "v"((int)(tid * 8u)), "s"(r), "s"((int)(c * 8u))
                 : "memory");
    return x;
  }
  template <int N>
  static __device__ __forceinline__ void pinned_wait(uint64_t (&x)[IOG])
  {
    static_assert(IOG == 4, "operand list");
    asm volatile("s_waitcnt vmcnt(%4)" : "+v"(x[0]), "+v"(x[1]), "+v"(x[2]), "+v"(x[3]) : "n"(N) : "memory");
  }
  template <int LOGN>
  __device__ __forceinline__ void store_prefetch(unsigned tid, StorePrefetch& pre) const
  {
// ... 29 lines not shown
          put(tid, eval_const<LOGN>(i), norm_from<12, EST>(shoup4_acc(cb[g & 1][j], cf, qc.nq, qc.q8 - x), qc));
        }
      });
      HX_SCHED_FENCE();
    });
  }
  __device__ __forceinline__ void put(unsigned tid, unsigned c, uint64_t o) const
  {
    asm volatile("buffer_store_dwordx2 %0, %1, %2, %3 offen" HX_NT_ASM
                 :
                 : "v"(o), "v"((int)(tid * 8u)), "s"(ro), "s"((int)(c * 8u))
                 : "memory");
  }
  __device__ __forceinline__ TW last_tw(TW def, int) const { return def; }
  __device__ __forceinline__ TWM last_tw(TWM def, int) const { return def; }
};


template <int LOGN, bool INV, class AR, class IO>
__device__ __forceinline__ void ntt_body_ar(uint32_t* lds, const IO& io, const typename AR::Tw* tw, const QC& q)
{
  using R = RowNTT<LOGN, AR>;
  uint64_t v[32];
  uint32_t nl[32];
  const unsigned w = wave_index();
  if constexpr (!INV) {
    R::template fwd<0>(fresh_tid(w), v, nl, lds, io, tw, q);
    __syncthreads();
    R::template fwd<1>(fresh_tid(w), v, nl, lds, io, tw, q);
    __syncthreads();
    R::template fwd<2>(fresh_tid(w), v, nl, lds, io, tw, q);
    __syncthreads();
    R::template fwd<3>(fresh_tid(w), v, nl, lds, io, tw, q);
    __syncthreads();
    R::template fwd<4>(fresh_tid(w), v, nl, lds, io, tw, q);
    __syncthreads();
    R::template fwd<5>(fresh_tid(w), v, nl, lds, io, tw, q);
    __syncthreads();
    R::template fwd<6>(fresh_tid(w), v, nl, lds, io, tw, q);
    __syncthreads();
    R::template fwd<7>(fresh_tid(w), v, nl, lds, io, tw, q);
  } else {
    R::template inv<0>(fresh_tid(w), v, nl, lds, io, tw, q);
    __syncthreads();
    R::template inv<1>(fresh_tid(w), v, nl, lds, io, tw, q);
    __syncthreads();
    R::template inv<2>(fresh_tid(w), v, nl, lds, io, tw, q);
    __syncthreads();
    R::template inv<3>(fresh_tid(w), v, nl, lds, io, tw, q);
    __syncthreads();
    R::template inv<4>(fresh_tid(w), v, nl, lds, io, tw, q);
    __syncthreads();
    R::template inv<5>(fresh_tid(w), v, nl, lds, io, tw, q);
    __syncthreads();
    R::template inv<6>(fresh_tid(w), v, nl, lds, io, tw, q);
    __syncthreads();
    R::template inv<7>(fresh_tid(w), v, nl, lds, io, tw, q);
  }
}
template <int LOGN, bool INV, class IO>
__device__ __forceinline__ void ntt_body(uint32_t* lds, const IO& io, const TW* tw_ptr, const PrimeDev* pd)
{
  const QC q = make_qc(pd->q, pd->mu64);
#ifndef HX_NO_PROTH
  if (pd->proth) {
    ntt_body_ar<LOGN, INV, ArProth>(lds, io, reinterpret_cast<const TWM*>(tw_ptr), q);
    return;
  }
#endif
  ntt_body_ar<LOGN, INV, ArShoup>(lds, io, tw_ptr, q);
}

template <int LOGN>
__global__ void __launch_bounds__(Geo<LOGN>::T, HX_NTT_MINWAVES(LOGN))
ntt_moddown_prep_kernel(PolyBases polys, int row, int prime, int batch, ModDownPrep P,
                        const PrimeDev* __restrict__ primes, const TW* __restrict__ tw_arena)
{
  extern __shared__ __attribute__((aligned(16))) uint32_t lds[];
  const int b = (int)(blockIdx.x % (unsigned)batch), pi = (int)(blockIdx.x / (unsigned)batch);
  const PrimeDev* pd = primes + prime;
  const size_t N = Geo<LOGN>::N;
  const uint64_t* in = poly_base(polys, (unsigned)pi);
  const size_t pstride = P.poly_stride ? (size_t)P.poly_stride : (size_t)batch * N;
  const InvPrepIO io(in + ((size_t)row * batch + b) * N, P, (size_t)pi * pstride + (size_t)b * N,
                     (unsigned)N * 8u);
  ntt_body<LOGN, true>(lds, io, tw_arena + pd->tw_inv_off, pd);
}
template <int LOGN>
__global__ void __launch_bounds__(Geo<LOGN>::T, HX_NTT_MINWAVES(LOGN))
ntt_moddown_prep_multi_kernel(PolyBases polys, PrepMulti M, int batch, ModDownPrep P,
                              const PrimeDev* __restrict__ primes, const TW* __restrict__ tw_arena)
{
  extern __shared__ __attribute__((aligned(16))) uint32_t lds[];
  const unsigned per = (unsigned)polys.n * (unsigned)batch;
  const unsigned j = blockIdx.x / per, rem = blockIdx.x % per;
  const int b = (int)(rem % (unsigned)batch), pi = (int)(rem / (unsigned)batch);
  const PrimeDev* pd = primes + uniform_u16(M.prime, j);
  const int row = (int)uniform_u16(M.row, j);
  const size_t N = Geo<LOGN>::N;
  const uint64_t* in = poly_base(polys, (unsigned)pi);
  ModDownPrep Pj = P;
  Pj.xs = P.xs + (size_t)j * (size_t)batch * N;
  Pj.upS = M.up[2 * j];
  Pj.upN = M.up[2 * j + 1];
  const InvPrepIO io(in + ((size_t)row * batch + b) * N, Pj, (size_t)pi * (size_t)P.poly_stride + (size_t)b * N,
                     (unsigned)N * 8u);
  ntt_body<LOGN, true>(lds, io, tw_arena + pd->tw_inv_off, pd);
}
template <int LOGN, bool PLAIN>
__global__ void __launch_bounds__(Geo<LOGN>::T, HX_NTT_MINWAVES(LOGN))
ntt_moddown_apply_kernel(PolyBases polys, PolyBases outs, NttRows rows, int nkeep, int batch, ModDownApply A,
                         const PrimeDev* __restrict__ primes, const TW* __restrict__ tw_arena)
{
  extern __shared__ __attribute__((aligned(16))) uint32_t lds[];
#ifdef HX_MD_OLDMAP
  const unsigned wid = xcd_remap(blockIdx.x, gridDim.x);
  const int b = (int)(wid % (unsigned)batch);
  const unsigned rp = wid / (unsigned)batch;
  const unsigned pi = rp % (unsigned)polys.n, ri = rp / (unsigned)polys.n;
#else
  const MdWork Wk = md_work(blockIdx.x, (unsigned)nkeep, (unsigned)polys.n * (unsigned)batch);
  if (!Wk.active)
    return;
  const unsigned ri = Wk.ri, pb = Wk.pb;
  const int b = (int)(pb % (unsigned)batch);
  const unsigned pi = pb / (unsigned)batch;
#endif
  const PrimeDev* pd = primes + uniform_u16(rows.prime, ri);
  const size_t N = Geo<LOGN>::N;
  const ModDownRow R = A.rows[ri];
  uint64_t* odata = poly_base(outs, pi);
  const uint64_t* idata = R.mode == 2 ? odata : poly_base(polys, pi);
  const size_t eoff = ((size_t)pi * batch + b) * N;
  const uint64_t* xrow = PLAIN ? A.delta + (size_t)pi * (size_t)A.delta_poly_stride + ((size_t)ri * batch + b) * N
                               : A.xs + eoff;
  const ModDownIO<PLAIN> io(xrow, PLAIN ? nullptr : A.S + eoff, R,
                            idata + ((size_t)(R.mode == 2 ? R.out_row : uniform_u16(rows.row, ri)) * batch + b) * N,
                            odata + ((size_t)R.out_row * batch + b) * N, (unsigned)N * 8u, pd->q);
  ntt_body<LOGN, false>(lds, io, tw_arena + pd->tw_fwd_off, pd);
}

__device__ __forceinline__ uint64_t tensor_red128(u128 S, uint64_t q, uint64_t mu63, uint32_t k)
{
  const uint64_t xt = (uint64_t)(S >> (k - 1));
  const uint32_t xl = (uint32_t)xt, xh = (uint32_t)(xt >> 32);
  const uint32_t ml = (uint32_t)mu63, mh = (uint32_t)(mu63 >> 32);
  const uint64_t qh = (uint64_t)xh * mh + __umulhi(xh, ml) + __umulhi(xl, mh);
  uint64_t r = (uint64_t)S - qh * q;
  r = csub(r, q << 2);
  r = csub(r, q << 1);
  return csub(r, q);
}
__device__ __forceinline__ uint64_t tensor_value(unsigned part, uint64_t a0, uint64_t a1, uint64_t b0, uint64_t b1,
                                                 uint64_t q, uint64_t mu, uint32_t k)
{
  if (part == 1)
    return tensor_red128((u128)a0 * b1 + (u128)a1 * b0, q, mu, k);
  return tensor_red128((u128)a0 * b0, q, mu, k);
}
struct InvPrepTensorIO {
  static constexpr int LOAD_BOUND = 1;
  static constexpr bool LAZY_STORE = false;
  static constexpr bool PIPELINED = false;
  struct StorePrefetch {};
  v4i32 ra, rb, rc, rd, rx;
  TW upS, upN;
  uint32_t has_up, part, k;
  uint64_t q, mu;
  __device__ InvPrepTensorIO(const TensorSrc& T, unsigned part_, size_t roff, const ModDownPrep& p, size_t xoff,
                             unsigned bytes, const PrimeDev* pd)
      : ra(make_rsrc((part_ == 2 ? T.a1 : T.a0) + roff, bytes)),
        rb(make_rsrc((part_ == 0 ? T.b0 : T.b1) + roff, bytes)),
        rc(make_rsrc(T.a1 + roff, bytes)), rd(make_rsrc(T.b0 + roff, bytes)),
        rx(make_rsrc(p.xs + xoff, bytes)), upS(p.upS), upN(p.upN), has_up(p.has_up), part(part_), k(pd->k), q(pd->q),
        mu(pd->mu63)
  {
  }
  static __device__ __forceinline__ uint64_t ld(const v4i32& r, unsigned tid, unsigned c)
  {
    v2i32 a = hx_buffer_load_v2(r, (int)(tid * 8u), (int)(c * 8u), 0);
    return ((uint64_t)(uint32_t)a.y << 32) | (uint32_t)a.x;
  }
  __device__ __forceinline__ uint64_t load(unsigned tid, unsigned c) const
  {
    const uint64_t x = ld(ra, tid, c), y = ld(rb, tid, c);
    if (part == 1)
      return tensor_value(1, x, ld(rc, tid, c), ld(rd, tid, c), y, q, mu, k);
    return tensor_value(0, x, 0, y, 0, q, mu, k);
  }
  __device__ __forceinline__ void store(unsigned tid, unsigned c, uint64_t x) const
  {
    v2i32 d;
    d.x = (int)(uint32_t)x;
    d.y = (int)(uint32_t)(x >> 32);
    hx_buffer_store_v2(d, rx, (int)(tid * 8u), (int)(c * 8u), 0);
  }
  __device__ __forceinline__ TW last_tw(TW def, int which) const { return has_up ? (which ? upN : upS) : def; }
  __device__ __forceinline__ TWM last_tw(TWM def, int which) const { return has_up ? (which ? upN.wp : upS.wp) : def; }
};
template <int LOGN>
__global__ void __launch_bounds__(Geo<LOGN>::T, HX_NTT_MINWAVES(LOGN))
ntt_moddown_prep_tensor_kernel(TensorSrc T, int row, int prime, int batch, ModDownPrep P,
                               const PrimeDev* __restrict__ primes, const TW* __restrict__ tw_arena)
{
  extern __shared__ __attribute__((aligned(16))) uint32_t lds[];
  const int b = (int)(blockIdx.x % (unsigned)batch), pi = (int)(blockIdx.x / (unsigned)batch);
  const PrimeDev* pd = primes + prime;
  const size_t N = Geo<LOGN>::N;
  const InvPrepTensorIO io(T, (unsigned)pi, ((size_t)row * batch + b) * N, P, ((size_t)pi * batch + b) * N,
                           (unsigned)N * 8u, pd);
  ntt_body<LOGN, true>(lds, io, tw_arena + pd->tw_inv_off, pd);
}

template <int LOGN>
__global__ void __launch_bounds__(Geo<LOGN>::T, HX_NTT_MINWAVES(LOGN))
ntt_moddown_prep_multi_tensor_kernel(TensorSrc T, PrepMulti M, int batch, ModDownPrep P,
                                     const PrimeDev* __restrict__ primes, const TW* __restrict__ tw_arena)
{
  extern __shared__ __attribute__((aligned(16))) uint32_t lds[];
  const unsigned per = 3u * (unsigned)batch;
  const unsigned j = blockIdx.x / per, rem = blockIdx.x % per;
  const int b = (int)(rem % (unsigned)batch), pi = (int)(rem / (unsigned)batch);
  const PrimeDev* pd = primes + uniform_u16(M.prime, j);
  const int row = (int)uniform_u16(M.row, j);
  const size_t N = Geo<LOGN>::N;
  ModDownPrep Pj = P;
  Pj.xs = P.xs + (size_t)j * (size_t)batch * N;
  Pj.upS = M.up[2 * j];
  Pj.upN = M.up[2 * j + 1];
  const InvPrepTensorIO io(T, (unsigned)pi, ((size_t)row * batch + b) * N, Pj,
                           (size_t)pi * (size_t)P.poly_stride + (size_t)b * N, (unsigned)N * 8u, pd);
  ntt_body<LOGN, true>(lds, io, tw_arena + pd->tw_inv_off, pd);
}

template <bool PLAIN>
struct ModDownTensorIO {
  static constexpr int LOAD_BOUND = PLAIN ? 8 : 6;
  template <class AR>
#ifndef HX_DIGITS_LB8
  static constexpr int load_bound() { return AR::PROTH ? 4 : (PLAIN ? 8 : 6); }
#else
  static constexpr int load_bound() { return PLAIN ? 8 : (AR::PROTH ? 4 : 6); }
#endif
  static constexpr bool LAZY_STORE = true;
  static constexpr bool PIPELINED = !PLAIN;
  static constexpr int IOG = 4;
  struct StorePrefetch {};
  v4i32 rx, rS, ra, rb, rc, rd, ro;
  TW inv, cf;
  uint64_t cf_r2;
  uint64_t q, mu;
  uint32_t part, k;
  __device__ ModDownTensorIO(const uint64_t* x_row, const int64_t* S_row, const ModDownRow& R, const TensorSrc& T,
                             unsigned part_, size_t roff, bool has_row, uint64_t* o_row, unsigned bytes, const PrimeDev* pd)
      : rx(make_rsrc(x_row, bytes)), rS(make_rsrc((const uint64_t*)S_row, bytes)),
        ra(make_rsrc(has_row ? (part_ == 2 ? T.a1 : T.a0) + roff : o_row, bytes)),
        rb(make_rsrc(has_row ? (part_ == 0 ? T.b0 : T.b1) + roff : o_row, bytes)),
        rc(make_rsrc(has_row ? T.a1 + roff : o_row, bytes)), rd(make_rsrc(has_row ? T.b0 + roff : o_row, bytes)),
        ro(make_rsrc(o_row, bytes)), inv(R.inv), cf(R.cf), cf_r2(R.cf_r2), q(pd->q), mu(pd->mu63), part(part_), k(pd->k)
  {
  }
  static __device__ __forceinline__ uint64_t ld(const v4i32& r, unsigned tid, unsigned c)
  {
    v2i32 a = hx_buffer_load_v2(r, (int)(tid * 8u), (int)(c * 8u), 0);
    return ((uint64_t)(uint32_t)a.y << 32) | (uint32_t)a.x;
  }
  __device__ __forceinline__ uint64_t load(unsigned tid, unsigned c) const
  {
    v2i32 a = hx_buffer_load_v2(rx, (int)(tid * 8u), (int)(c * 8u), HX_NT);
    return ((uint64_t)(uint32_t)a.y << 32) | (uint32_t)a.x;
  }
  template <int LOGN, class AR>
  __device__ __forceinline__ void load_all(unsigned tid, uint64_t (&v)[32], const QC& qc) const
  {
    static_for<0, 32>([&](auto E) {
      constexpr int e = decltype(E)::value;
      v[e] = ld(rx, tid, coef_const<LOGN>(e));
    });
    uint64_t sb[2][IOG];
    static_for<0, IOG>([&](auto J) {
      constexpr int j = decltype(J)::value;
      sb[0][j] = ld(rS, tid, coef_const<LOGN>(j));
    });
    HX_SCHED_FENCE();
    static_for<0, 32 / IOG>([&](auto GI) {
      constexpr int g = decltype(GI)::value;
      if constexpr (g + 1 < 32 / IOG)
        static_for<0, IOG>([&](auto J) {
          constexpr int j = decltype(J)::value;
          sb[(g + 1) & 1][j] = ld(rS, tid, coef_const<LOGN>((g + 1) * IOG + j));
        });
      static_for<0, IOG>([&](auto J) {
        constexpr int j = decltype(J)::value, e = g * IOG + j;
        if constexpr (AR::PROTH)
          v[e] = mont_acc(v[e], inv.wp, qc, q - sb[g & 1][j]);
        else
          v[e] = shoup4_acc(v[e], inv, qc.nq, q - sb[g & 1][j]);
      });
      HX_SCHED_FENCE();
    });
  }
  static __device__ __forceinline__ uint64_t ld_pinned(const v4i32& r, unsigned tid, unsigned c)
  {
    uint64_t x;
    asm volatile("buffer_load_dwordx2 %0, %1, %2, %3 offen" : "=v"(x) : "v"((int)(tid * 8u)), "s"(r), "s"((int)(c * 8u)) : "memory");
    return x;
  }
  template <int N>
  static __device__ __forceinline__ void pinned_wait(uint64_t (&x)[8])
  {
    asm volatile("s_waitcnt vmcnt(%8)"
                 : "+v"(x[0]), "+v"(x[1]), "+v"(x[2]), "+v"(x[3]), "+v"(x[4]), "+v"(x[5]), "+v"(x[6]), "+v"(x[7])
                 : "n"(N)
                 : "memory");
// ... 131 lines not shown
#endif
  ntt_body<LOGN, INV>(lds, io, tw, pd);
}

template <bool PROTH>
struct MulLoadIO {
  static constexpr int LOAD_BOUND = 1;
  static constexpr bool LAZY_STORE = false;
  static constexpr bool PIPELINED = false;
  template <class AR>
  static constexpr int inv_load_bound() { return PROTH ? 2 : 1; }
  struct StorePrefetch {};
  v4i32 ra, rb, ro;
  uint64_t q, mu63, r2;
  uint32_t k;
  __device__ MulLoadIO(const uint64_t* a_row, const uint64_t* b_row, uint64_t* o_row, unsigned bytes, const PrimeDev* pd)
      : ra(make_rsrc(a_row, bytes)), rb(make_rsrc(b_row, bytes)), ro(make_rsrc(o_row, bytes)), q(pd->q), mu63(pd->mu63),
        r2(pd->r2), k(pd->k)
  {
  }
  __device__ __forceinline__ uint64_t load(unsigned tid, unsigned c) const
  {
    const v2i32 x = hx_buffer_load_v2(ra, (int)(tid * 8u), (int)(c * 8u), HX_NT);
    const v2i32 y = hx_buffer_load_v2(rb, (int)(tid * 8u), (int)(c * 8u), HX_NT);
    const uint64_t a = ((uint64_t)(uint32_t)x.y << 32) | (uint32_t)x.x, b = ((uint64_t)(uint32_t)y.y << 32) | (uint32_t)y.x;
    const u128 p = (u128)a * b;
    if constexpr (PROTH)
      return mont_redc128((uint64_t)p, (uint64_t)(p >> 64), make_qc(q, 0));
    else
      return tensor_red128(p, q, mu63, k);
  }
  __device__ __forceinline__ void store(unsigned tid, unsigned c, uint64_t v) const
  {
    v2i32 d;
    d.x = (int)(uint32_t)v;
    d.y = (int)(uint32_t)(v >> 32);
    hx_buffer_store_v2(d, ro, (int)(tid * 8u), (int)(c * 8u), HX_NT);
  }
  __device__ __forceinline__ TW last_tw(TW def, int) const { return def; }
  __device__ __forceinline__ TWM last_tw(TWM def, int) const
  {
    if constexpr (PROTH) {
      const QC qc = make_qc(q, 0);
      return csub(mont_mul(def, r2, qc), q);
    } else {
      return def;
    }
  }
};
template <int LOGN>
__global__ void __launch_bounds__(Geo<LOGN>::T, HX_NTT_MINWAVES(LOGN))
ntt_inv_mul_kernel(const uint64_t* a, const uint64_t* b, uint64_t* out, NttRows rows, int batch,
                   const PrimeDev* __restrict__ primes, const TW* __restrict__ tw_arena)
{
  extern __shared__ __attribute__((aligned(16))) uint32_t lds[];
  const unsigned wid = xcd_remap(blockIdx.x, gridDim.x);
  const unsigned ri = wid / (unsigned)batch;
  const int bb = (int)(wid % (unsigned)batch);
  const int row = (int)uniform_u16(rows.row, ri);
  const PrimeDev* pd = primes + uniform_u16(rows.prime, ri);
  const size_t N = Geo<LOGN>::N;
  const size_t roff = ((size_t)row * batch + bb) * N, ooff = ((size_t)ri * batch + bb) * N;
  const QC qc = make_qc(pd->q, pd->mu64);
  const TW* tw = tw_arena + pd->tw_inv_off;
#ifndef HX_NO_PROTH
  if (pd->proth) {
#ifndef HX_INVMUL_BARRETT
    const MulLoadIO<true> io(a + roff, b + roff, out + ooff, (unsigned)N * 8u, pd);
#else
    const MulLoadIO<false> io(a + roff, b + roff, out + ooff, (unsigned)N * 8u, pd);
#endif
    ntt_body_ar<LOGN, true, ArProth>(lds, io, reinterpret_cast<const TWM*>(tw), qc);
    return;
  }
#endif
  const MulLoadIO<false> io(a + roff, b + roff, out + ooff, (unsigned)N * 8u, pd);
  ntt_body_ar<LOGN, true, ArShoup>(lds, io, tw, qc);
}
template <int LOGN>
static hipError_t launch_inv_mul(const uint64_t* a, const uint64_t* b, uint64_t* out, const NttRows& rows, int nrows,
                                 int batch, const PrimeDev* primes, const TW* tw_arena, hipStream_t st)
{
  constexpr size_t lds_bytes = (size_t)Geo<LOGN>::LDS_WORDS * 4;
  bool attr_set = false;
  if (!attr_set) {
    hipError_t e = hxp::dyn_lds((const void*)ntt_inv_mul_kernel<LOGN>, (int)lds_bytes);
    if (e != hipSuccess)
      return e;
    attr_set = true;
  }
  HX_LAUNCH((ntt_inv_mul_kernel<LOGN>), dim3((unsigned)nrows * (unsigned)batch), dim3(Geo<LOGN>::T), lds_bytes, st, a, b,
            out, rows, batch, primes, tw_arena);
  return hipGetLastError();
}
hipError_t HX_ENTRY(launch_ntt_inv_mul_pow2)(int logn, const uint64_t* a, const uint64_t* b, uint64_t* out, const NttRows& rows,
                                   int nrows, int batch, const PrimeDev* primes, const TW* tw_arena, hipStream_t st)
{
  switch (logn) {
    HX_SZ(13, launch_inv_mul<13>(a, b, out, rows, nrows, batch, primes, tw_arena, st))
    HX_SZ(14, launch_inv_mul<14>(a, b, out, rows, nrows, batch, primes, tw_arena, st))
    HX_SZ(15, launch_inv_mul<15>(a, b, out, rows, nrows, batch, primes, tw_arena, st))
  }
  return hipErrorInvalidValue;
}

template <int LOGN, bool INV, int LB = 1>
static hipError_t launch_one(const uint64_t* in, uint64_t* out, const NttRows& rows, int nrows,
                             int batch, const PrimeDev* primes, const TW* tw_arena, hipStream_t st)
{
#ifdef HX_ROW_ONE_WG
  static const size_t lds_bytes = LOGN == 14 ? (size_t)90 * 1024 : (size_t)Geo<LOGN>::LDS_WORDS * 4;
#else
  static const size_t lds_bytes = (size_t)Geo<LOGN>::LDS_WORDS * 4;
#endif
  bool attr_set = false;
  if (!attr_set) {
    hipError_t e = hxp::dyn_lds((const void*)ntt_row_kernel<LOGN, INV, LB>,
                                       hipFuncAttributeMaxDynamicSharedMemorySize, (int)lds_bytes);
    if (e != hipSuccess)
      return e;
    attr_set = true;
  }
  dim3 grid((unsigned)nrows * (unsigned)batch), block(Geo<LOGN>::T);
  HX_LAUNCH((ntt_row_kernel<LOGN, INV, LB>), grid, block, lds_bytes, st, in, out, rows, batch,
                     primes, tw_arena);
  return hipGetLastError();
}

template <int LOGN>
static hipError_t moddown_attrs()
{
  constexpr size_t lds_bytes = (size_t)Geo<LOGN>::LDS_WORDS * 4;
  bool attr_set = false;
  if (!attr_set) {
    hipError_t e = hxp::dyn_lds((const void*)ntt_moddown_prep_kernel<LOGN>, (int)lds_bytes);
    if (e == hipSuccess)
      e = hxp::dyn_lds((const void*)ntt_moddown_prep_multi_kernel<LOGN>, (int)lds_bytes);
    if (e == hipSuccess)
      e = hxp::dyn_lds((const void*)ntt_moddown_apply_kernel<LOGN, false>,
                              hipFuncAttributeMaxDynamicSharedMemorySize, (int)lds_bytes);
    if (e == hipSuccess)
      e = hxp::dyn_lds((const void*)ntt_moddown_apply_kernel<LOGN, true>,
                              hipFuncAttributeMaxDynamicSharedMemorySize, (int)lds_bytes);
    if (e != hipSuccess)
      return e;
    attr_set = true;
  }
  return hipSuccess;
}
static unsigned moddown_apply_grid(unsigned npoly, unsigned nkeep, unsigned batch)
{
#ifdef HX_MD_OLDMAP
  return npoly * nkeep * batch;
#else
  return 8u * md_tile(nkeep, npoly * batch).per_xcd;
#endif
}

template <int LOGN>
static hipError_t launch_moddown(const PolyBases& polys, const PolyBases& outs, int drop_row, int drop_prime,
                                 const NttRows& keep, int nkeep, int batch, const ModDownPrep& P,
                                 const ModDownApply& A, const PrimeDev* primes, const TW* tw_arena,
                                 hipStream_t st)
{
  constexpr size_t lds_bytes = (size_t)Geo<LOGN>::LDS_WORDS * 4;
  hipError_t e = moddown_attrs<LOGN>();
  if (e != hipSuccess)
    return e;
  HX_LAUNCH((ntt_moddown_prep_kernel<LOGN>), dim3((unsigned)polys.n * (unsigned)batch),
                     dim3(Geo<LOGN>::T), lds_bytes, st, polys, drop_row, drop_prime, batch, P, primes,
                     tw_arena);
  {
    const size_t n = (size_t)polys.n * (size_t)batch * Geo<LOGN>::N;
    HX_LAUNCH((moddown_S_kernel<0>), dim3((unsigned)((n / 2 + 255) / 256 > 8192 ? 8192 : (n / 2 + 255) / 256)),
                       dim3(256), 0, st, P, n / 2);
  }
  HX_LAUNCH((ntt_moddown_apply_kernel<LOGN, false>),
                     dim3(moddown_apply_grid((unsigned)polys.n, (unsigned)nkeep, (unsigned)batch)),
                     dim3(Geo<LOGN>::T), lds_bytes, st, polys, outs, keep, nkeep, batch, A, primes, tw_arena);
  return hipGetLastError();
}

hipError_t HX_ENTRY(launch_moddown_pow2)(int logn, const PolyBases& data, const PolyBases& out, int drop_row,
                               int drop_prime, const NttRows& keep, int nkeep, int batch,
                               const ModDownPrep& P, const ModDownApply& A, const PrimeDev* primes,
                               const TW* tw_arena, hipStream_t st)
{
  switch (logn) {
    HX_SZ(13, launch_moddown<13>(data, out, drop_row, drop_prime, keep, nkeep, batch, P, A, primes, tw_arena, st))
    HX_SZ(14, launch_moddown<14>(data, out, drop_row, drop_prime, keep, nkeep, batch, P, A, primes, tw_arena, st))
    HX_SZ(15, launch_moddown<15>(data, out, drop_row, drop_prime, keep, nkeep, batch, P, A, primes, tw_arena, st))
  }
  return hipErrorInvalidValue;
}

template <int LOGN>
static hipError_t moddown_tensor_attrs()
{
  constexpr size_t lds_bytes = (size_t)Geo<LOGN>::LDS_WORDS * 4;
  bool attr_set = false;
  if (!attr_set) {
    hipError_t e = hxp::dyn_lds((const void*)ntt_moddown_prep_tensor_kernel<LOGN>, (int)lds_bytes);
    if (e == hipSuccess)
      e = hxp::dyn_lds((const void*)ntt_moddown_prep_multi_tensor_kernel<LOGN>, (int)lds_bytes);
    if (e == hipSuccess)
      e = hxp::dyn_lds((const void*)ntt_moddown_apply_tensor_kernel<LOGN, false>,
                              hipFuncAttributeMaxDynamicSharedMemorySize, (int)lds_bytes);
    if (e == hipSuccess)
      e = hxp::dyn_lds((const void*)ntt_moddown_apply_tensor_kernel<LOGN, true>,
                              hipFuncAttributeMaxDynamicSharedMemorySize, (int)lds_bytes);
    if (e != hipSuccess)
      return e;
    attr_set = true;
  }
  return hipSuccess;
}
template <int LOGN>
static hipError_t launch_moddown_tensor(const TensorSrc& T, const PolyBases& outs, int drop_row, int drop_prime,
                                        const NttRows& keep, int nkeep, int batch, const ModDownPrep& P,
                                        const ModDownApply& A, const PrimeDev* primes, const TW* tw_arena, hipStream_t st)
{
  constexpr size_t lds_bytes = (size_t)Geo<LOGN>::LDS_WORDS * 4;
  hipError_t ea = moddown_tensor_attrs<LOGN>();
  if (ea != hipSuccess)
    return ea;
  HX_LAUNCH((ntt_moddown_prep_tensor_kernel<LOGN>), dim3(3u * (unsigned)batch), dim3(Geo<LOGN>::T), lds_bytes, st, T,
            drop_row, drop_prime, batch, P, primes, tw_arena);
  {
    const size_t n = (size_t)3 * (size_t)batch * Geo<LOGN>::N;
    HX_LAUNCH((moddown_S_kernel<0>), dim3((unsigned)((n / 2 + 255) / 256 > 8192 ? 8192 : (n / 2 + 255) / 256)), dim3(256), 0, st, P,
              n / 2);
  }
  HX_LAUNCH((ntt_moddown_apply_tensor_kernel<LOGN, false>), dim3(moddown_apply_grid(3u, (unsigned)nkeep, (unsigned)batch)),
            dim3(Geo<LOGN>::T), lds_bytes, st, T, outs, keep, nkeep, batch, A, primes, tw_arena);
  return hipGetLastError();
}
hipError_t HX_ENTRY(launch_moddown_tensor_pow2)(int logn, const TensorSrc& T, const PolyBases& outs, int drop_row, int drop_prime,
                                      const NttRows& keep, int nkeep, int batch, const ModDownPrep& P,
                                      const ModDownApply& A, const PrimeDev* primes, const TW* tw_arena, hipStream_t st)
{
  switch (logn) {
    HX_SZ(13, launch_moddown_tensor<13>(T, outs, drop_row, drop_prime, keep, nkeep, batch, P, A, primes, tw_arena, st))
    HX_SZ(14, launch_moddown_tensor<14>(T, outs, drop_row, drop_prime, keep, nkeep, batch, P, A, primes, tw_arena, st))
    HX_SZ(15, launch_moddown_tensor<15>(T, outs, drop_row, drop_prime, keep, nkeep, batch, P, A, primes, tw_arena, st))
  }
  return hipErrorInvalidValue;
}

template <int LOGN>
static hipError_t launch_prep_multi_tensor(const TensorSrc& T, const PrepMulti& M, int ndrop, int batch, const ModDownPrep& P,
                                           const PrimeDev* primes, const TW* tw_arena, hipStream_t st)
{
  constexpr size_t lds_bytes = (size_t)Geo<LOGN>::LDS_WORDS * 4;
  hipError_t e = moddown_tensor_attrs<LOGN>();
  if (e != hipSuccess)
    return e;
  HX_LAUNCH((ntt_moddown_prep_multi_tensor_kernel<LOGN>), dim3((unsigned)ndrop * 3u * (unsigned)batch), dim3(Geo<LOGN>::T),
            lds_bytes, st, T, M, batch, P, primes, tw_arena);
  return hipGetLastError();
}
template <int LOGN>
static hipError_t launch_apply_plain_tensor(const TensorSrc& T, const PolyBases& outs, const NttRows& keep, int nkeep,
                                            int batch, const ModDownApply& A, const PrimeDev* primes, const TW* tw_arena,
                                            hipStream_t st)
{
  constexpr size_t lds_bytes = (size_t)Geo<LOGN>::LDS_WORDS * 4;
  hipError_t e = moddown_tensor_attrs<LOGN>();
  if (e != hipSuccess)
    return e;
  HX_LAUNCH((ntt_moddown_apply_tensor_kernel<LOGN, true>), dim3(moddown_apply_grid(3u, (unsigned)nkeep, (unsigned)batch)),
            dim3(Geo<LOGN>::T), lds_bytes, st, T, outs, keep, nkeep, batch, A, primes, tw_arena);
  return hipGetLastError();
}
hipError_t HX_ENTRY(launch_moddown_prep_multi_tensor_pow2)(int logn, const TensorSrc& T, const PrepMulti& M, int ndrop, int batch,
                                                 const ModDownPrep& P, const PrimeDev* primes, const TW* tw_arena,
                                                 hipStream_t st)
{
  switch (logn) {
    HX_SZ(13, launch_prep_multi_tensor<13>(T, M, ndrop, batch, P, primes, tw_arena, st))
    HX_SZ(14, launch_prep_multi_tensor<14>(T, M, ndrop, batch, P, primes, tw_arena, st))
    HX_SZ(15, launch_prep_multi_tensor<15>(T, M, ndrop, batch, P, primes, tw_arena, st))
  }
  return hipErrorInvalidValue;
}
hipError_t HX_ENTRY(launch_moddown_apply_plain_tensor_pow2)(int logn, const TensorSrc& T, const PolyBases& outs, const NttRows& keep,
                                                  int nkeep, int batch, const ModDownApply& A, const PrimeDev* primes,
                                                  const TW* tw_arena, hipStream_t st)
{
  switch (logn) {
    HX_SZ(13, launch_apply_plain_tensor<13>(T, outs, keep, nkeep, batch, A, primes, tw_arena, st))
    HX_SZ(14, launch_apply_plain_tensor<14>(T, outs, keep, nkeep, batch, A, primes, tw_arena, st))
    HX_SZ(15, launch_apply_plain_tensor<15>(T, outs, keep, nkeep, batch, A, primes, tw_arena, st))
  }
  return hipErrorInvalidValue;
}

template <int LOGN>
static hipError_t launch_prep_one(const PolyBases& polys, int drop_row, int drop_prime, int batch,
                                  const ModDownPrep& P, const PrimeDev* primes, const TW* tw_arena, hipStream_t st)
{
  constexpr size_t lds_bytes = (size_t)Geo<LOGN>::LDS_WORDS * 4;
  hipError_t e = moddown_attrs<LOGN>();
  if (e != hipSuccess)
    return e;
  HX_LAUNCH((ntt_moddown_prep_kernel<LOGN>), dim3((unsigned)polys.n * (unsigned)batch),
                     dim3(Geo<LOGN>::T), lds_bytes, st, polys, drop_row, drop_prime, batch, P, primes,
                     tw_arena);
  return hipGetLastError();
}
template <int LOGN>
static hipError_t launch_apply_plain(const PolyBases& polys, const PolyBases& outs, const NttRows& keep,
                                     int nkeep, int batch, const ModDownApply& A, const PrimeDev* primes,
                                     const TW* tw_arena, hipStream_t st)
{
  constexpr size_t lds_bytes = (size_t)Geo<LOGN>::LDS_WORDS * 4;
// ... 236 lines not shown
```

helib_amd/csrc/prof.h:

```cpp
#pragma once
#include <hip/hip_runtime.h>
#include <hip/hip_ext.h>

#include <cxxabi.h>
#include <algorithm>
#include <atomic>
#include <cstdio>
#include <cstdlib>
#include <map>
#include <mutex>
#include <string>
#include <unordered_map>
#include <vector>

namespace hxp {

inline hipError_t dyn_lds(const void* kern, int bytes)
{
  static std::mutex mu;
  static std::map<std::pair<int, const void*>, int> done;
  int dev = 0;
  hipError_t e = hipGetDevice(&dev);
  if (e != hipSuccess)
    return e;
  std::lock_guard<std::mutex> lk(mu);
  auto it = done.find({dev, kern});
  if (it != done.end() && it->second >= bytes)
    return hipSuccess;
  e = hipFuncSetAttribute(kern, hipFuncAttributeMaxDynamicSharedMemorySize, bytes);
  if (e == hipSuccess)
    done[{dev, kern}] = bytes;
  return e;
}
inline hipError_t dyn_lds(const void* kern, hipFuncAttribute, int bytes) { return dyn_lds(kern, bytes); }

struct Rec {
  int name, device;
  unsigned wgs, wg_size;
  hipEvent_t e0, e1;
};
struct State {
  std::mutex mu;
  std::vector<std::string> names;
  std::unordered_map<const void*, int> by_ptr;
  std::vector<Rec> recs;
  std::map<int, std::vector<hipEvent_t>> spare;
  size_t dropped = 0;
  std::string summary;
  bool have_summary = false;
};
inline std::atomic<bool> enabled{false};
inline State& state()
{
  static State s;
  return s;
}
static constexpr size_t MAX_RECS = (size_t)1 << 18;

inline hipEvent_t take_event(State& s, int device)
{
  hipEvent_t e = nullptr;
  std::vector<hipEvent_t>& pool = s.spare[device];
  if (!pool.empty()) {
    e = pool.back();
    pool.pop_back();
  } else if (hipEventCreate(&e) != hipSuccess) {
    (void)hipGetLastError();
    e = nullptr;
  }
  return e;
}

inline bool pre(const void* fn, const char* text, hipStream_t st, dim3 grid, dim3 block, hipEvent_t* e0, hipEvent_t* e1)
{
  State& s = state();
  std::lock_guard<std::mutex> lk(s.mu);
  hipStreamCaptureStatus cs = hipStreamCaptureStatusNone;
  if (hipStreamIsCapturing(st, &cs) != hipSuccess) {
    (void)hipGetLastError();
    return false;
  }
  if (cs != hipStreamCaptureStatusNone)
    return false;
  if (s.recs.size() >= MAX_RECS) {
    s.dropped++;
    return false;
  }
  auto it = s.by_ptr.find(fn);
  if (it == s.by_ptr.end()) {
    std::string nm;
    const char* mangled = hipKernelNameRefByPtr(fn, st);
    if (mangled) {
      int status = 0;
      char* dem = abi::__cxa_demangle(mangled, nullptr, nullptr, &status);
      nm = (status == 0 && dem) ? dem : mangled;
      free(dem);
    } else {
      (void)hipGetLastError();
      nm = text;
    }
    const size_t paren = nm.find('(');
    if (paren != std::string::npos && paren > 0)
      nm.resize(paren);
    if (nm.rfind("void ", 0) == 0)
      nm.erase(0, 5);
    s.names.push_back(nm);
    it = s.by_ptr.emplace(fn, (int)s.names.size() - 1).first;
  }
  Rec r;
  r.name = it->second;
  r.device = 0;
  if (hipGetDevice(&r.device) != hipSuccess)
    (void)hipGetLastError();
  r.wgs = grid.x * grid.y * grid.z;
// ... 112 lines not shown
```

Baseline: 43600 mult/s.

## Fuse moddown S computation into prep NTT store and add lock-free LDS attribute cache

The separate moddown_S_kernel launch (unless HX_MD_S_KERNEL is defined) is removed. The inverse-NTT prep kernels now write both xs and S in their store phase, using a compile-time variant chosen by plaintext-modulus class. This saves one full read pass over xs and one kernel launch per mod-down. Separately, dyn_lds drops its per-call hipGetDevice, mutex and map lookup in favour of a thread-local current device plus a lock-free hash table, which cuts host overhead on every launch. The cost is more register pressure and extra stores inside the NTT epilogue.

```diff
diff --git a/helib_amd/csrc/bgv_slots.hip b/helib_amd/csrc/bgv_slots.hip
--- a/helib_amd/csrc/bgv_slots.hip
+++ b/helib_amd/csrc/bgv_slots.hip
@@ -182,7 +182,7 @@
 {
   if (!t)
     return HX_OK;
-  (void)hipSetDevice(t->device);
+  (void)hxp::set_device(t->device);
   if (t->side)
     hx_ctx_destroy(t->side);
   hipFree(t->d_row2slot);
diff --git a/helib_amd/csrc/conv_kernels.hip b/helib_amd/csrc/conv_kernels.hip
--- a/helib_amd/csrc/conv_kernels.hip
+++ b/helib_amd/csrc/conv_kernels.hip
@@ -203,14 +203,9 @@
                               const TW* tw_arena, hipStream_t st)
 {
   constexpr size_t lds_bytes = (size_t)Geo<LOGN>::LDS_WORDS * 4;
-  bool attr_set = false;
-  if (!attr_set) {
-    hipError_t e = hxp::dyn_lds((const void*)ntt_conv_kernel<LOGN, SRC, DST>,
-                                       hipFuncAttributeMaxDynamicSharedMemorySize, (int)lds_bytes);
-    if (e != hipSuccess)
-      return e;
-    attr_set = true;
-  }
+  const hipError_t e = hxp::dyn_lds((const void*)ntt_conv_kernel<LOGN, SRC, DST>, (int)lds_bytes);
+  if (e != hipSuccess)
+    return e;
   HX_LAUNCH((ntt_conv_kernel<LOGN, SRC, DST>), dim3((unsigned)nunits * A.batch), dim3(Geo<LOGN>::T), lds_bytes, st, A, R,
             cprimes, tw_arena);
   return hipGetLastError();
diff --git a/helib_amd/csrc/engine.hip b/helib_amd/csrc/engine.hip
--- a/helib_amd/csrc/engine.hip
+++ b/helib_amd/csrc/engine.hip
@@ -262,7 +262,7 @@
 
 static int use(hx_ctx* c)
 {
-  HIPCHK(hipSetDevice(c->device));
+  HIPCHK(hxp::set_device(c->device));
   return HX_OK;
 }
 #define CTX_ENTER(ctx)                                             \
@@ -444,7 +444,7 @@
     return fail(HX_ERR_DEVICE, "no HIP device available (this library has no CPU path)");
   if (device < 0 || device >= ndev)
     return fail(HX_ERR_INVALID, "device %d out of range [0,%d)", device, ndev);
-  HIPCHK(hipSetDevice(device));
+  HIPCHK(hxp::set_device(device));
   hx_ctx* c = new hx_ctx();
   c->sw = hxs::read();
   struct Guard {
@@ -502,7 +502,7 @@
 }
 static void ctx_free(hx_ctx* c)
 {
-  hipSetDevice(c->device);
+  hxp::set_device(c->device);
   hipDeviceSynchronize();
   if (c->ckks_free)
     c->ckks_free(c->ckks);
@@ -594,7 +594,7 @@
   if (c->capturing)
     return fail(HX_ERR_INVALID, "hx_ctx_set_stream while a graph is being captured");
   if (c->stream != (hipStream_t)s) {
-    hipSetDevice(c->device);
+    hxp::set_device(c->device);
     hipStreamSynchronize(c->stream);
     if (c->norm_stream)
       hipStreamSynchronize(c->norm_stream);
@@ -1622,7 +1622,7 @@
     return HX_OK;
   {
     std::lock_guard<std::recursive_mutex> lk(p->ctx->mu);
-    hipSetDevice(p->ctx->device);
+    hxp::set_device(p->ctx->device);
     storage_release(p);
     p->ctx->polys.erase(p);
   }
@@ -1655,7 +1655,7 @@
   if (!p)
     return nullptr;
   std::lock_guard<std::recursive_mutex> lk(p->ctx->mu);
-  hipSetDevice(p->ctx->device);
+  hxp::set_device(p->ctx->device);
   if (poly_own(p) != HX_OK)
     return nullptr;
   p->exposed = true;
@@ -2122,7 +2122,7 @@
   hx_ctx* c = g->ctx;
   {
     std::lock_guard<std::recursive_mutex> lk(c->mu);
-    hipSetDevice(c->device);
+    hxp::set_device(c->device);
     hipStreamSynchronize(c->stream);
     hipGraphExecDestroy(g->exec);
     hipGraphDestroy(g->graph);
@@ -2672,18 +2672,10 @@
     }
     const dim3 wgrid((unsigned)((row_words + hx::WIDE_THREADS - 1) / hx::WIDE_THREADS)), wblock(hx::WIDE_THREADS);
     const size_t lds = wide_lds;
-    static std::mutex wide_mu;
-    static std::unordered_set<int> wide_attr;
-    {
-      std::lock_guard<std::mutex> lk(wide_mu);
-      if (!wide_attr.count(c->device)) {
-        for (const void* f : {(const void*)hx::rns_extend_wide_kernel<20>, (const void*)hx::rns_extend_wide_kernel<24>,
-                              (const void*)hx::rns_extend_wide_kernel<28>, (const void*)hx::rns_extend_wide_kernel<32>,
-                              (const void*)hx::rns_extend_wide_kernel<36>, (const void*)hx::rns_extend_wide_kernel<40>})
-          HIPCHK(hxp::dyn_lds(f, 160 * 1024));
-        wide_attr.insert(c->device);
-      }
-    }
+    for (const void* f : {(const void*)hx::rns_extend_wide_kernel<20>, (const void*)hx::rns_extend_wide_kernel<24>,
+                          (const void*)hx::rns_extend_wide_kernel<28>, (const void*)hx::rns_extend_wide_kernel<32>,
+                          (const void*)hx::rns_extend_wide_kernel<36>, (const void*)hx::rns_extend_wide_kernel<40>})
+      HIPCHK(hxp::dyn_lds(f, 160 * 1024));
     if (n <= 20)
       HX_LAUNCH((hx::rns_extend_wide_kernel<20>), wgrid, wblock, lds, c->stream, pl->dev, args, row_words);
     else if (n <= 24)
@@ -2813,12 +2805,8 @@
   HIPCHK(hipMemcpy(c->d_bn_v, v.data(), sizeof(double) * 2 * m, hipMemcpyHostToDevice));
   HIPCHK(hipMemcpy(c->d_bn_w, w.data(), sizeof(double) * P, hipMemcpyHostToDevice));
   HIPCHK(hipMemcpy(d_cv, cv.data(), sizeof(double) * 2 * P, hipMemcpyHostToDevice));
-  bool attr = false;
-  if (!attr) {
-    HIPCHK(hxp::dyn_lds((const void*)hx::bnorm_fwd_kernel, 16 << hx::NORM_MAX_LOGH));
-    HIPCHK(hxp::dyn_lds((const void*)hx::bnorm_inv_kernel, 16 << hx::NORM_MAX_LOGH));
-    attr = true;
-  }
+  HIPCHK(hxp::dyn_lds((const void*)hx::bnorm_fwd_kernel, 16 << hx::NORM_MAX_LOGH));
+  HIPCHK(hxp::dyn_lds((const void*)hx::bnorm_inv_kernel, 16 << hx::NORM_MAX_LOGH));
   const int logp = bk, logh = std::min(logp, hx::NORM_MAX_LOGH);
   const unsigned H = 1u << logh, S = (unsigned)(P >> logh);
   const unsigned threads = std::min<unsigned>(hx::NORM_THREADS, std::max<unsigned>(64u, H / 4));
@@ -2950,11 +2938,10 @@
   unsigned long long* const out2 = direct ? np.pinned : c->d_norm2;
   if (!direct)
     HIPCHK(hipMemsetAsync(c->d_norm2, 0, sizeof(unsigned long long) * (size_t)rows, ns));
-  bool attr = false;
   if (!c->pow2) {
     CHK(flush_xs(c));
     CHK(embed_norms_general(c, d_f, rows, ns));
-  } else if (!attr) {
+  } else {
     HIPCHK(hxp::dyn_lds((const void*)hx::embed_norm_kernel, 16 << hx::NORM_MAX_LOGH));
 #define HX_NORM_ATTR(...)                                                                               \
   HIPCHK(hxp::dyn_lds((const void*)hx::embed_norm_quarter_kernel<__VA_ARGS__>,                   \
@@ -2967,7 +2954,6 @@
     HX_NORM_ATTR(hx::NormSrcXS, 14);
 #undef HX_NORM_ATTR
     HIPCHK(hxp::dyn_lds((const void*)hx::embed_norm_quarter_split_kernel, 16 << hx::NORM_MAX_LOGH));
-    attr = true;
   }
   if (!c->pow2) {
   } else if (logn >= 2 && logn - 1 <= hx::NORM_MAX_LOGH) {
@@ -2990,12 +2976,8 @@
     const bool r16 = !c->sw.norm_old;
     constexpr size_t r16_lds = (size_t)hx::R16_LDS_DOUBLES * sizeof(double);
     if (r16 && logn == 14) {
-      bool attr16 = false;
-      if (!attr16) {
-        HIPCHK(hxp::dyn_lds((const void*)hx::embed_norm_r16_kernel<hx::NormSrcXS>, (int)r16_lds));
-        HIPCHK(hxp::dyn_lds((const void*)hx::embed_norm_r16_kernel<hx::NormSrcF64>, (int)r16_lds));
-        attr16 = true;
-      }
+      HIPCHK(hxp::dyn_lds((const void*)hx::embed_norm_r16_kernel<hx::NormSrcXS>, (int)r16_lds));
+      HIPCHK(hxp::dyn_lds((const void*)hx::embed_norm_r16_kernel<hx::NormSrcF64>, (int)r16_lds));
     }
     if (c->xs_rows == rows && d_f == c->d_frac) {
       hx::NormSrcXS src{c->scratch[0], reinterpret_cast<const int64_t*>(c->scratch[1]), c->xs_inv_qd};
@@ -3030,11 +3012,7 @@
     }
     if (x2) {
       constexpr size_t x2_lds = 2 * (size_t)hx::R16_LDS_DOUBLES * sizeof(double);
-      bool attrx2 = false;
-      if (!attrx2) {
-        HIPCHK(hxp::dyn_lds((const void*)hx::embed_norm_r16x2_kernel, (int)x2_lds));
-        attrx2 = true;
-      }
+      HIPCHK(hxp::dyn_lds((const void*)hx::embed_norm_r16x2_kernel, (int)x2_lds));
       HX_LAUNCH(hx::embed_norm_r16x2_kernel, dim3((unsigned)rows), dim3(2 * hx::R16_THREADS), x2_lds, ns, d_f, c->d_wtab,
                 out2, direct);
     } else
@@ -4084,18 +4062,10 @@
     }
 #undef HX_BRK_LAUNCH
   } else if (nmax <= 8) {
-    bool attr8 = false;
-    if (!attr8) {
-      HIPCHK(hxp::dyn_lds((const void*)hx::break_digits_kernel<8>, 64 * hx::BRK_THREADS * 8));
-      attr8 = true;
-    }
+    HIPCHK(hxp::dyn_lds((const void*)hx::break_digits_kernel<8>, 64 * hx::BRK_THREADS * 8));
     HX_LAUNCH((hx::break_digits_kernel<8>), grid, block, lds, c->stream, A, rw);
   } else {
-    bool attr16 = false;
-    if (!attr16) {
-      HIPCHK(hxp::dyn_lds((const void*)hx::break_digits_kernel<16>, 64 * hx::BRK_THREADS * 8));
-      attr16 = true;
-    }
+    HIPCHK(hxp::dyn_lds((const void*)hx::break_digits_kernel<16>, 64 * hx::BRK_THREADS * 8));
     HX_LAUNCH((hx::break_digits_kernel<16>), grid, block, lds, c->stream, A, rw);
   }
   HIPCHK(hipGetLastError());
@@ -4220,7 +4190,7 @@
 {
   if (!k)
     return HX_OK;
-  hipSetDevice(k->ctx->device);
+  hxp::set_device(k->ctx->device);
   hipStreamSynchronize(k->ctx->stream);
   hipFree(k->d_b);
   hipFree(k->d_a);
diff --git a/helib_amd/csrc/ntt_core.h b/helib_amd/csrc/ntt_core.h
--- a/helib_amd/csrc/ntt_core.h
+++ b/helib_amd/csrc/ntt_core.h
@@ -747,6 +747,11 @@
 struct io_inv_load_bound<IO, AR, std::void_t<decltype(IO::template inv_load_bound<AR>())>>
     : std::integral_constant<int, IO::template inv_load_bound<AR>()> {};
 
+template <class IO, class = void>
+struct io_store_variants : std::false_type {};
+template <class IO>
+struct io_store_variants<IO, std::void_t<decltype(IO::STORE_VARIANTS)>> : std::integral_constant<bool, IO::STORE_VARIANTS> {};
+
 struct PtrIO {
   static constexpr int LOAD_BOUND = 1;
   static constexpr bool LAZY_STORE = false;
@@ -950,10 +955,20 @@
             HX_SCHED_FENCE();
         });
       }
-#pragma unroll
-      for (int e = 0; e < 32; e++) {
-        io.store(tid, coef_const<LOGN>(e), norm_from<AR::INV_OUT>(v[e], c));
-        HX_IO_FENCE(e);
+      if constexpr (io_store_variants<IO>::value) {
+        io.store_variant([&](auto V) {
+#pragma unroll
+          for (int e = 0; e < 32; e++) {
+            io.template store_as<decltype(V)::value>(tid, coef_const<LOGN>(e), norm_from<AR::INV_OUT>(v[e], c));
+            HX_IO_FENCE(e);
+          }
+        });
+      } else {
+#pragma unroll
+        for (int e = 0; e < 32; e++) {
+          io.store(tid, coef_const<LOGN>(e), norm_from<AR::INV_OUT>(v[e], c));
+          HX_IO_FENCE(e);
+        }
       }
     }
   }
diff --git a/helib_amd/csrc/ntt_kernels.hip b/helib_amd/csrc/ntt_kernels.hip
--- a/helib_amd/csrc/ntt_kernels.hip
+++ b/helib_amd/csrc/ntt_kernels.hip
@@ -106,53 +106,20 @@
   __device__ __forceinline__ TWM last_tw(TWM def, int) const { return def; }
 };
 
-struct InvPrepIO {
-  static constexpr int LOAD_BOUND = 1;
-  static constexpr bool LAZY_STORE = false;
-  static constexpr bool PIPELINED = false;
-  struct StorePrefetch {};
-  v4i32 rin, rx;
-  TW upS, upN;
-  uint32_t has_up;
-  __device__ InvPrepIO(const uint64_t* in_row, const ModDownPrep& p, size_t boff, unsigned bytes)
-      : rin(make_rsrc(in_row, bytes)), rx(make_rsrc(p.xs + boff, bytes)), upS(p.upS), upN(p.upN),
-        has_up(p.has_up)
-  {
-  }
-  __device__ __forceinline__ uint64_t load(unsigned tid, unsigned c) const
-  {
-    v2i32 r = hx_buffer_load_v2(rin, (int)(tid * 8u), (int)(c * 8u), HX_NT);
-    return ((uint64_t)(uint32_t)r.y << 32) | (uint32_t)r.x;
-  }
-  __device__ __forceinline__ void store(unsigned tid, unsigned c, uint64_t x) const
-  {
-    v2i32 d;
-    d.x = (int)(uint32_t)x;
-    d.y = (int)(uint32_t)(x >> 32);
-    hx_buffer_store_v2(d, rx, (int)(tid * 8u), (int)(c * 8u), 0);
-  }
-  __device__ __forceinline__ TW last_tw(TW def, int which) const
-  {
-    return has_up ? (which ? upN : upS) : def;
-  }
-  __device__ __forceinline__ TWM last_tw(TWM def, int which) const
-  {
-    return has_up ? (which ? upN.wp : upS.wp) : def;
-  }
-};
-
+constexpr int MD_PTXT_ONE = 0, MD_PTXT_WORD = 1, MD_PTXT_WIDE = 2;
+template <int CLS = -1>
 __device__ __forceinline__ int64_t moddown_S_of(const ModDownPrep& P, uint64_t x)
 {
   const bool neg = x > P.half;
   int64_t S = neg ? 1 : 0;
-  if (P.ptxt > 1) {
+  if (CLS < 0 ? P.ptxt > 1 : CLS != MD_PTXT_ONE) {
     const uint64_t p = P.ptxt;
     uint64_t r = red64(x, p, P.ptxt_mu64);
     if (neg)
       r = sub_mod(r, P.qd_mod_p, p);
     if (r != 0) {
-      const uint64_t dm = (p >> 32) == 0 ? red64(r * P.qdinv_mod_p, p, P.ptxt_mu64)
-                                         : mul_mod(r, P.qdinv_mod_p, p, P.ptxt_mu, P.ptxt_k);
+      const uint64_t dm = (CLS < 0 ? (p >> 32) == 0 : CLS == MD_PTXT_WORD) ? red64(r * P.qdinv_mod_p, p, P.ptxt_mu64)
+                                                                            : mul_mod(r, P.qdinv_mod_p, p, P.ptxt_mu, P.ptxt_k);
       const uint64_t p2 = p >> 1;
       const bool sub_p = dm > p2 || (((p & 1) == 0) && dm == p2 && neg);
       S += sub_p ? (int64_t)dm - (int64_t)p : (int64_t)dm;
@@ -160,6 +127,8 @@
   }
   return S;
 }
+#ifdef HX_MD_S_KERNEL
+constexpr bool MD_PREP_FORMS_S = false;
 template <int UNUSED = 0>
 __global__ void __launch_bounds__(256)
 moddown_S_kernel(ModDownPrep P, size_t n2)
@@ -174,6 +143,68 @@
     S[i] = s;
   }
 }
+static void launch_moddown_S(const ModDownPrep& P, size_t n, hipStream_t st)
+{
+  HX_LAUNCH((moddown_S_kernel<0>), dim3((unsigned)((n / 2 + 255) / 256 > 8192 ? 8192 : (n / 2 + 255) / 256)), dim3(256), 0,
+            st, P, n / 2);
+}
+#else
+constexpr bool MD_PREP_FORMS_S = true;
+#endif
+
+template <bool WITH_S>
+struct InvPrepStore {
+  static constexpr bool STORE_VARIANTS = WITH_S;
+  v4i32 rx, rS;
+  const ModDownPrep& P;
+  __device__ InvPrepStore(const ModDownPrep& p, size_t off, unsigned bytes)
+      : rx(make_rsrc(p.xs + off, bytes)), rS(WITH_S ? make_rsrc(reinterpret_cast<const uint64_t*>(p.S) + off, bytes) : rx), P(p)
+  {
+  }
+  static __device__ __forceinline__ void put(const v4i32& r, unsigned tid, unsigned c, uint64_t x)
+  {
+    v2i32 d;
+    d.x = (int)(uint32_t)x;
+    d.y = (int)(uint32_t)(x >> 32);
+    hx_buffer_store_v2(d, r, (int)(tid * 8u), (int)(c * 8u), 0);
+  }
+  __device__ __forceinline__ void store(unsigned tid, unsigned c, uint64_t x) const { put(rx, tid, c, x); }
+  template <class F>
+  __device__ __forceinline__ void store_variant(F&& loop) const
+  {
+    if (P.ptxt <= 1)
+      loop(std::integral_constant<int, MD_PTXT_ONE>{});
+    else if ((P.ptxt >> 32) == 0)
+      loop(std::integral_constant<int, MD_PTXT_WORD>{});
+    else
+      loop(std::integral_constant<int, MD_PTXT_WIDE>{});
+  }
+  template <int CLS>
+  __device__ __forceinline__ void store_as(unsigned tid, unsigned c, uint64_t x) const
+  {
+    put(rx, tid, c, x);
+    put(rS, tid, c, (uint64_t)moddown_S_of<CLS>(P, x));
+  }
+  __device__ __forceinline__ TW last_tw(TW def, int which) const { return P.has_up ? (which ? P.upN : P.upS) : def; }
+  __device__ __forceinline__ TWM last_tw(TWM def, int which) const { return P.has_up ? (which ? P.upN.wp : P.upS.wp) : def; }
+};
+template <bool WITH_S>
+struct InvPrepIO : InvPrepStore<WITH_S> {
+  static constexpr int LOAD_BOUND = 1;
+  static constexpr bool LAZY_STORE = false;
+  static constexpr bool PIPELINED = false;
+  struct StorePrefetch {};
+  v4i32 rin;
+  __device__ InvPrepIO(const uint64_t* in_row, const ModDownPrep& p, size_t boff, unsigned bytes)
+      : InvPrepStore<WITH_S>(p, boff, bytes), rin(make_rsrc(in_row, bytes))
+  {
+  }
+  __device__ __forceinline__ uint64_t load(unsigned tid, unsigned c) const
+  {
+    v2i32 r = hx_buffer_load_v2(rin, (int)(tid * 8u), (int)(c * 8u), HX_NT);
+    return ((uint64_t)(uint32_t)r.y << 32) | (uint32_t)r.x;
+  }
+};
 
 template <bool PLAIN>
 struct ModDownIO {
@@ -369,8 +400,8 @@
   const size_t N = Geo<LOGN>::N;
   const uint64_t* in = poly_base(polys, (unsigned)pi);
   const size_t pstride = P.poly_stride ? (size_t)P.poly_stride : (size_t)batch * N;
-  const InvPrepIO io(in + ((size_t)row * batch + b) * N, P, (size_t)pi * pstride + (size_t)b * N,
-                     (unsigned)N * 8u);
+  const InvPrepIO<MD_PREP_FORMS_S> io(in + ((size_t)row * batch + b) * N, P, (size_t)pi * pstride + (size_t)b * N,
+                                      (unsigned)N * 8u);
   ntt_body<LOGN, true>(lds, io, tw_arena + pd->tw_inv_off, pd);
 }
 template <int LOGN>
@@ -390,8 +421,8 @@
   Pj.xs = P.xs + (size_t)j * (size_t)batch * N;
   Pj.upS = M.up[2 * j];
   Pj.upN = M.up[2 * j + 1];
-  const InvPrepIO io(in + ((size_t)row * batch + b) * N, Pj, (size_t)pi * (size_t)P.poly_stride + (size_t)b * N,
-                     (unsigned)N * 8u);
+  const InvPrepIO<false> io(in + ((size_t)row * batch + b) * N, Pj, (size_t)pi * (size_t)P.poly_stride + (size_t)b * N,
+                            (unsigned)N * 8u);
   ntt_body<LOGN, true>(lds, io, tw_arena + pd->tw_inv_off, pd);
 }
 template <int LOGN, bool PLAIN>
@@ -445,21 +476,20 @@
     return tensor_red128((u128)a0 * b1 + (u128)a1 * b0, q, mu, k);
   return tensor_red128((u128)a0 * b0, q, mu, k);
 }
-struct InvPrepTensorIO {
+template <bool WITH_S>
+struct InvPrepTensorIO : InvPrepStore<WITH_S> {
   static constexpr int LOAD_BOUND = 1;
   static constexpr bool LAZY_STORE = false;
   static constexpr bool PIPELINED = false;
   struct StorePrefetch {};
-  v4i32 ra, rb, rc, rd, rx;
-  TW upS, upN;
-  uint32_t has_up, part, k;
+  v4i32 ra, rb, rc, rd;
+  uint32_t part, k;
   uint64_t q, mu;
   __device__ InvPrepTensorIO(const TensorSrc& T, unsigned part_, size_t roff, const ModDownPrep& p, size_t xoff,
                              unsigned bytes, const PrimeDev* pd)
-      : ra(make_rsrc((part_ == 2 ? T.a1 : T.a0) + roff, bytes)),
+      : InvPrepStore<WITH_S>(p, xoff, bytes), ra(make_rsrc((part_ == 2 ? T.a1 : T.a0) + roff, bytes)),
         rb(make_rsrc((part_ == 0 ? T.b0 : T.b1) + roff, bytes)),
-        rc(make_rsrc(T.a1 + roff, bytes)), rd(make_rsrc(T.b0 + roff, bytes)),
-        rx(make_rsrc(p.xs + xoff, bytes)), upS(p.upS), upN(p.upN), has_up(p.has_up), part(part_), k(pd->k), q(pd->q),
+        rc(make_rsrc(T.a1 + roff, bytes)), rd(make_rsrc(T.b0 + roff, bytes)), part(part_), k(pd->k), q(pd->q),
         mu(pd->mu63)
   {
   }
@@ -475,15 +505,6 @@
       return tensor_value(1, x, ld(rc, tid, c), ld(rd, tid, c), y, q, mu, k);
     return tensor_value(0, x, 0, y, 0, q, mu, k);
   }
-  __device__ __forceinline__ void store(unsigned tid, unsigned c, uint64_t x) const
-  {
-    v2i32 d;
-    d.x = (int)(uint32_t)x;
-    d.y = (int)(uint32_t)(x >> 32);
-    hx_buffer_store_v2(d, rx, (int)(tid * 8u), (int)(c * 8u), 0);
-  }
-  __device__ __forceinline__ TW last_tw(TW def, int which) const { return has_up ? (which ? upN : upS) : def; }
-  __device__ __forceinline__ TWM last_tw(TWM def, int which) const { return has_up ? (which ? upN.wp : upS.wp) : def; }
 };
 template <int LOGN>
 __global__ void __launch_bounds__(Geo<LOGN>::T, HX_NTT_MINWAVES(LOGN))
@@ -494,8 +515,8 @@
   const int b = (int)(blockIdx.x % (unsigned)batch), pi = (int)(blockIdx.x / (unsigned)batch);
   const PrimeDev* pd = primes + prime;
   const size_t N = Geo<LOGN>::N;
-  const InvPrepTensorIO io(T, (unsigned)pi, ((size_t)row * batch + b) * N, P, ((size_t)pi * batch + b) * N,
-                           (unsigned)N * 8u, pd);
+  const InvPrepTensorIO<MD_PREP_FORMS_S> io(T, (unsigned)pi, ((size_t)row * batch + b) * N, P, ((size_t)pi * batch + b) * N,
+                                            (unsigned)N * 8u, pd);
   ntt_body<LOGN, true>(lds, io, tw_arena + pd->tw_inv_off, pd);
 }
 
@@ -515,8 +536,8 @@
   Pj.xs = P.xs + (size_t)j * (size_t)batch * N;
   Pj.upS = M.up[2 * j];
   Pj.upN = M.up[2 * j + 1];
-  const InvPrepTensorIO io(T, (unsigned)pi, ((size_t)row * batch + b) * N, Pj,
-                           (size_t)pi * (size_t)P.poly_stride + (size_t)b * N, (unsigned)N * 8u, pd);
+  const InvPrepTensorIO<false> io(T, (unsigned)pi, ((size_t)row * batch + b) * N, Pj,
+                                  (size_t)pi * (size_t)P.poly_stride + (size_t)b * N, (unsigned)N * 8u, pd);
   ntt_body<LOGN, true>(lds, io, tw_arena + pd->tw_inv_off, pd);
 }
 
@@ -814,13 +835,9 @@
                                  int batch, const PrimeDev* primes, const TW* tw_arena, hipStream_t st)
 {
   constexpr size_t lds_bytes = (size_t)Geo<LOGN>::LDS_WORDS * 4;
-  bool attr_set = false;
-  if (!attr_set) {
-    hipError_t e = hxp::dyn_lds((const void*)ntt_inv_mul_kernel<LOGN>, (int)lds_bytes);
-    if (e != hipSuccess)
-      return e;
-    attr_set = true;
-  }
+  const hipError_t e = hxp::dyn_lds((const void*)ntt_inv_mul_kernel<LOGN>, (int)lds_bytes);
+  if (e != hipSuccess)
+    return e;
   HX_LAUNCH((ntt_inv_mul_kernel<LOGN>), dim3((unsigned)nrows * (unsigned)batch), dim3(Geo<LOGN>::T), lds_bytes, st, a, b,
             out, rows, batch, primes, tw_arena);
   return hipGetLastError();
@@ -845,14 +862,9 @@
 #else
   static const size_t lds_bytes = (size_t)Geo<LOGN>::LDS_WORDS * 4;
 #endif
-  bool attr_set = false;
-  if (!attr_set) {
-    hipError_t e = hxp::dyn_lds((const void*)ntt_row_kernel<LOGN, INV, LB>,
-                                       hipFuncAttributeMaxDynamicSharedMemorySize, (int)lds_bytes);
-    if (e != hipSuccess)
-      return e;
-    attr_set = true;
-  }
+  const hipError_t e = hxp::dyn_lds((const void*)ntt_row_kernel<LOGN, INV, LB>, (int)lds_bytes);
+  if (e != hipSuccess)
+    return e;
   dim3 grid((unsigned)nrows * (unsigned)batch), block(Geo<LOGN>::T);
   HX_LAUNCH((ntt_row_kernel<LOGN, INV, LB>), grid, block, lds_bytes, st, in, out, rows, batch,
                      primes, tw_arena);
@@ -863,22 +875,14 @@
 static hipError_t moddown_attrs()
 {
   constexpr size_t lds_bytes = (size_t)Geo<LOGN>::LDS_WORDS * 4;
-  bool attr_set = false;
-  if (!attr_set) {
-    hipError_t e = hxp::dyn_lds((const void*)ntt_moddown_prep_kernel<LOGN>, (int)lds_bytes);
-    if (e == hipSuccess)
-      e = hxp::dyn_lds((const void*)ntt_moddown_prep_multi_kernel<LOGN>, (int)lds_bytes);
-    if (e == hipSuccess)
-      e = hxp::dyn_lds((const void*)ntt_moddown_apply_kernel<LOGN, false>,
-                              hipFuncAttributeMaxDynamicSharedMemorySize, (int)lds_bytes);
-    if (e == hipSuccess)
-      e = hxp::dyn_lds((const void*)ntt_moddown_apply_kernel<LOGN, true>,
-                              hipFuncAttributeMaxDynamicSharedMemorySize, (int)lds_bytes);
-    if (e != hipSuccess)
-      return e;
-    attr_set = true;
-  }
-  return hipSuccess;
+  hipError_t e = hxp::dyn_lds((const void*)ntt_moddown_prep_kernel<LOGN>, (int)lds_bytes);
+  if (e == hipSuccess)
+    e = hxp::dyn_lds((const void*)ntt_moddown_prep_multi_kernel<LOGN>, (int)lds_bytes);
+  if (e == hipSuccess)
+    e = hxp::dyn_lds((const void*)ntt_moddown_apply_kernel<LOGN, false>, (int)lds_bytes);
+  if (e == hipSuccess)
+    e = hxp::dyn_lds((const void*)ntt_moddown_apply_kernel<LOGN, true>, (int)lds_bytes);
+  return e;
 }
 static unsigned moddown_apply_grid(unsigned npoly, unsigned nkeep, unsigned batch)
 {
@@ -902,11 +906,9 @@
   HX_LAUNCH((ntt_moddown_prep_kernel<LOGN>), dim3((unsigned)polys.n * (unsigned)batch),
                      dim3(Geo<LOGN>::T), lds_bytes, st, polys, drop_row, drop_prime, batch, P, primes,
                      tw_arena);
-  {
-    const size_t n = (size_t)polys.n * (size_t)batch * Geo<LOGN>::N;
-    HX_LAUNCH((moddown_S_kernel<0>), dim3((unsigned)((n / 2 + 255) / 256 > 8192 ? 8192 : (n / 2 + 255) / 256)),
-                       dim3(256), 0, st, P, n / 2);
-  }
+#ifdef HX_MD_S_KERNEL
+  launch_moddown_S(P, (size_t)polys.n * (size_t)batch * Geo<LOGN>::N, st);
+#endif
   HX_LAUNCH((ntt_moddown_apply_kernel<LOGN, false>),
                      dim3(moddown_apply_grid((unsigned)polys.n, (unsigned)nkeep, (unsigned)batch)),
                      dim3(Geo<LOGN>::T), lds_bytes, st, polys, outs, keep, nkeep, batch, A, primes, tw_arena);
@@ -930,22 +932,14 @@
 static hipError_t moddown_tensor_attrs()
 {
   constexpr size_t lds_bytes = (size_t)Geo<LOGN>::LDS_WORDS * 4;
-  bool attr_set = false;
-  if (!attr_set) {
-    hipError_t e = hxp::dyn_lds((const void*)ntt_moddown_prep_tensor_kernel<LOGN>, (int)lds_bytes);
-    if (e == hipSuccess)
-      e = hxp::dyn_lds((const void*)ntt_moddown_prep_multi_tensor_kernel<LOGN>, (int)lds_bytes);
-    if (e == hipSuccess)
-      e = hxp::dyn_lds((const void*)ntt_moddown_apply_tensor_kernel<LOGN, false>,
-                              hipFuncAttributeMaxDynamicSharedMemorySize, (int)lds_bytes);
-    if (e == hipSuccess)
-      e = hxp::dyn_lds((const void*)ntt_moddown_apply_tensor_kernel<LOGN, true>,
-                              hipFuncAttributeMaxDynamicSharedMemorySize, (int)lds_bytes);
-    if (e != hipSuccess)
-      return e;
-    attr_set = true;
-  }
-  return hipSuccess;
+  hipError_t e = hxp::dyn_lds((const void*)ntt_moddown_prep_tensor_kernel<LOGN>, (int)lds_bytes);
+  if (e == hipSuccess)
+    e = hxp::dyn_lds((const void*)ntt_moddown_prep_multi_tensor_kernel<LOGN>, (int)lds_bytes);
+  if (e == hipSuccess)
+    e = hxp::dyn_lds((const void*)ntt_moddown_apply_tensor_kernel<LOGN, false>, (int)lds_bytes);
+  if (e == hipSuccess)
+    e = hxp::dyn_lds((const void*)ntt_moddown_apply_tensor_kernel<LOGN, true>, (int)lds_bytes);
+  return e;
 }
 template <int LOGN>
 static hipError_t launch_moddown_tensor(const TensorSrc& T, const PolyBases& outs, int drop_row, int drop_prime,
@@ -958,11 +952,9 @@
     return ea;
   HX_LAUNCH((ntt_moddown_prep_tensor_kernel<LOGN>), dim3(3u * (unsigned)batch), dim3(Geo<LOGN>::T), lds_bytes, st, T,
             drop_row, drop_prime, batch, P, primes, tw_arena);
-  {
-    const size_t n = (size_t)3 * (size_t)batch * Geo<LOGN>::N;
-    HX_LAUNCH((moddown_S_kernel<0>), dim3((unsigned)((n / 2 + 255) / 256 > 8192 ? 8192 : (n / 2 + 255) / 256)), dim3(256), 0, st, P,
-              n / 2);
-  }
+#ifdef HX_MD_S_KERNEL
+  launch_moddown_S(P, (size_t)3 * (size_t)batch * Geo<LOGN>::N, st);
+#endif
   HX_LAUNCH((ntt_moddown_apply_tensor_kernel<LOGN, false>), dim3(moddown_apply_grid(3u, (unsigned)nkeep, (unsigned)batch)),
             dim3(Geo<LOGN>::T), lds_bytes, st, T, outs, keep, nkeep, batch, A, primes, tw_arena);
   return hipGetLastError();
diff --git a/helib_amd/csrc/prof.h b/helib_amd/csrc/prof.h
--- a/helib_amd/csrc/prof.h
+++ b/helib_amd/csrc/prof.h
@@ -5,6 +5,7 @@
 #include <cxxabi.h>
 #include <algorithm>
 #include <atomic>
+#include <cstdint>
 #include <cstdio>
 #include <cstdlib>
 #include <map>
@@ -15,21 +16,58 @@
 
 namespace hxp {
 
+inline thread_local int cur_device = -1;
+inline hipError_t set_device(int device)
+{
+  const hipError_t e = hipSetDevice(device);
+  cur_device = e == hipSuccess ? device : -1;
+  return e;
+}
+
+constexpr int LDS_MAX_DEV = 16, LDS_SLOTS = 512;
+struct LdsGrant {
+  std::atomic<const void*> kern{nullptr};
+  std::atomic<int> bytes[LDS_MAX_DEV] = {};
+};
+inline LdsGrant* lds_grants()
+{
+  static LdsGrant t[LDS_SLOTS];
+  return t;
+}
+inline LdsGrant* lds_slot(const void* kern)
+{
+  LdsGrant* t = lds_grants();
+  size_t h = ((uintptr_t)kern >> 4) * (size_t)0x9E3779B97F4A7C15ull >> 32;
+  for (int i = 0; i < LDS_SLOTS; i++, h++) {
+    LdsGrant* g = &t[h % LDS_SLOTS];
+    const void* k = g->kern.load(std::memory_order_acquire);
+    if (k == kern || k == nullptr)
+      return g;
+  }
+  return nullptr;
+}
 inline hipError_t dyn_lds(const void* kern, int bytes)
 {
+  const int dev = cur_device;
+  if (dev >= 0 && dev < LDS_MAX_DEV) {
+    const LdsGrant* g = lds_slot(kern);
+    if (g && g->kern.load(std::memory_order_relaxed) == kern && g->bytes[dev].load(std::memory_order_acquire) >= bytes)
+      return hipSuccess;
+  }
   static std::mutex mu;
-  static std::map<std::pair<int, const void*>, int> done;
-  int dev = 0;
-  hipError_t e = hipGetDevice(&dev);
+  std::lock_guard<std::mutex> lk(mu);
+  int now = 0;
+  hipError_t e = hipGetDevice(&now);
   if (e != hipSuccess)
     return e;
-  std::lock_guard<std::mutex> lk(mu);
-  auto it = done.find({dev, kern});
-  if (it != done.end() && it->second >= bytes)
-    return hipSuccess;
   e = hipFuncSetAttribute(kern, hipFuncAttributeMaxDynamicSharedMemorySize, bytes);
-  if (e == hipSuccess)
-    done[{dev, kern}] = bytes;
+  if (e != hipSuccess || now < 0 || now >= LDS_MAX_DEV)
+    return e;
+  if (LdsGrant* g = lds_slot(kern)) {
+    if (g->bytes[now].load(std::memory_order_relaxed) < bytes)
+      g->bytes[now].store(bytes, std::memory_order_release);
+    g->kern.store(kern, std::memory_order_release);
+  }
   return e;
 }
 inline hipError_t dyn_lds(const void* kern, hipFuncAttribute, int bytes) { return dyn_lds(kern, bytes); }
```

Result: no change. 43750 mult/s (median of 6 runs) (+0.3%).
